# DefaultRui/VLN-VER

Hardware: AMD Instinct MI355X
Metric: viewpoints/sec (multi-view->voxel fwd+bwd), vocc.py config (higher is better)
Workload: dtype bf16

## Files before the change

### include/ver_ops.h

```cpp
#ifndef VER_OPS_H
#define VER_OPS_H

#include <stdint.h>

#ifdef __cplusplus
extern "C" {
#endif

#define VER_ABI_VERSION 31

#define VER_OK            0
#define VER_EINVAL       -1
#define VER_EUNSUPPORTED -2
#define VER_ELAUNCH      -3

#define VER_F32  0
#define VER_BF16 1

#define VER_I32  0
#define VER_I64  1

int         ver_abi_version(void);
const char* ver_last_error(void);

int ver_msda_forward(const float* value, const int64_t* shapes_hw, const int64_t* level_start,
                     const float* loc, const float* attn_w, float* out,
                     int B, int num_keys, int heads, int head_dim, int levels, int points,
                     int Nq, int im2col_step, void* stream);

int ver_msda_backward(const float* value, const int64_t* shapes_hw, const int64_t* level_start,
                      const float* loc, const float* attn_w, const float* grad_out,
                      float* grad_value, float* grad_loc, float* grad_attn_w,
                      int B, int num_keys, int heads, int head_dim, int levels, int points,
                      int Nq, int im2col_step, void* stream);

int ver_msda3d_forward(const float* value, const int64_t* shapes_dhw, const int64_t* level_start,
                       const float* loc, const float* attn_w, float* out,
                       int B, int num_keys, int heads, int head_dim, int levels, int points,
                       int Nq, void* stream);
int ver_msda3d_backward(const float* value, const int64_t* shapes_dhw, const int64_t* level_start,
                        const float* loc, const float* attn_w, const float* grad_out,
                        float* grad_value, float* grad_loc, float* grad_attn_w,
                        int B, int num_keys, int heads, int head_dim, int levels, int points,
                        int Nq, void* stream);


int ver_project_points(const float* world2pixel, const float* origin, const float* pc_range,
                       int B, int Ncam, int bev_z, int bev_h, int bev_w,
                       float img_w, float img_h,
                       float* uv, uint8_t* vis, int32_t* vis_list, int32_t* vis_cnt,
                       int32_t* zero_list, int32_t* zero_cnt, int32_t* fwd_list, int32_t* fwd_cnt,
                       void* stream);

int ver_hits_from_mask(const uint8_t* bev_mask, int B, int Ncam, int Nq, int D,
                       uint8_t* vis, int32_t* vis_list, int32_t* vis_cnt,
                       int32_t* zero_list, int32_t* zero_cnt, int32_t* fwd_list, int32_t* fwd_cnt,
                       void* stream);

#define VER_SCA_ROWS_PREZEROED 1
#define VER_SCA_VALUE_HEAD_MAJOR 2
#define VER_SCA_GRAD_SLOTS_BF16 4
int ver_sca_head_major_supported(int value_dtype, int head_dim, int points, int map_h, int map_w);
int ver_sca_zero_rows(const int32_t* zero_list, const int32_t* zero_cnt, float* slots, int B, int Nq, int row_floats,
                      void* stream);
int ver_sca_forward(const void* value, int value_dtype, const float* offsets, const float* logits,
                    const float* uv, const uint8_t* vis, const int32_t* vis_list,
                    const int32_t* vis_cnt, const int32_t* zero_list, const int32_t* zero_cnt,
                    const int32_t* fwd_list, const int32_t* fwd_cnt,
                    float* slots,
                    int B, int Ncam, int Nq, int D, int heads, int head_dim, int points,
                    int map_h, int map_w, int flags, void* stream);

int ver_sca_backward_grad_dtype(int value_dtype, int head_dim, int points, int map_h, int map_w);
int ver_sca_backward(const void* value, int value_dtype, const float* offsets, const float* logits,
                     const float* uv, const uint8_t* vis, const int32_t* vis_list,
                     const int32_t* vis_cnt, const int32_t* fwd_list, const int32_t* fwd_cnt,
                     const void* grad_slots,
                     void* grad_value, int grad_value_dtype, float* grad_offsets, float* grad_logits,
                     int B, int Ncam, int Nq, int D, int heads, int head_dim, int points,
                     int map_h, int map_w, int flags, void* stream);

int ver_lattice_im2col(const void* src, void* col, const int* taps, int ntaps,
                       int B, int Z, int H, int W, int C, int dtype, void* stream);
int ver_lattice_col2im(const void* grad_col, void* grad_src, const int* taps, int ntaps,
                       int B, int Z, int H, int W, int C, int dtype, void* stream);

int ver_lattice_gather(const void* src, void* col, const int* taps, const long* col_offset, long col_stride,
                       int ntaps, int B, int Zr, int Zs, int H, int W, int C, int layout, int dtype,
                       const void* const_rows, const long* const_offset, int const_blocks, int const_width, void* stream);
int ver_lattice_scatter(const void* grad_col, void* grad_src, const int* taps, const long* col_offset,
                        long col_stride, int ntaps, int B, int Zr, int Zs, int H, int W, int C, int layout, int dtype,
                        void* stream);

int ver_convt_weight_forward(const float* weight, void* taps, long pairs, int dtype, void* stream);
int ver_convt_weight_backward(const void* grad_taps, float* grad_weight, long pairs, int dtype, void* stream);
int ver_convt_weight_backward_blocks(const void* blocks, const long* block_offsets, long ld, const void* prev_bias,
                                     const void* grad_v, float* grad_weight, int ci, int co, int dtype, void* stream);
int ver_convt_weight_forward_blocks(const float* weight, const long* block_offsets, long ld, void* blocks, int ci, int co,
                                    int dtype, void* stream);
int ver_blocks_vec_forward(const void* blocks, const long* block_rows, int nblocks, long ld, int ci, int ncols, const float* x,
                           float* vec, int dtype, void* stream);
int ver_blocks_vec_backward(const void* blocks, const long* block_rows, int nblocks, long ld, int ci, int ncols,
                            const float* grad_vec, float* grad_x, int dtype, void* stream);
int ver_lattice_transpose(void* channels_last, void* channel_first, long cf_stride, int B, int Z, int H, int W,
                          int C, int layout, int to_channel_first, int dtype, void* stream);
int ver_lattice_rows(void* channels_last, void* rows, long quarter, int period, int nseg, const int* seg_off,
                     const int* seg_len, const long* seg_base, const int* seg_pitch, const int* seg_rows, int B, int Z,
                     int H, int W, int C, int layout, int to_rows, int dtype, void* stream);

int ver_ln_relu_forward(const void* x, const float* gamma, const float* beta, void* y,
                        float* mean, float* rstd, long N, int W, float eps, int dtype, void* stream);
int ver_ln_relu_backward(const void* x, const void* grad_y, const float* gamma, const float* beta,
                         const float* mean, const float* rstd, void* grad_x,
                         float* grad_gamma, float* grad_beta, long N, int W, int dtype, void* stream);

int ver_focal_loss_blocks(long N, int C);
int ver_focal_loss_forward(const void* logits, const int64_t* target, float* partial, long N, int C,
                           float gamma, float alpha, int dtype, int32_t* bad_labels, void* stream);
int ver_focal_loss_forward_grad(const void* logits, const int64_t* target, float* partial, void* grad, long N, int C,
                                float gamma, float alpha, int dtype, int32_t* bad_labels, void* stream);
int ver_focal_loss_forward_grad_u8(const void* logits, const uint8_t* target, float* partial, void* grad, long N, int C,
                                   float gamma, float alpha, int dtype, int32_t* bad_labels, void* stream);
int ver_focal_loss_backward(const void* logits, const int64_t* target, const float* scale, void* grad,
                            long N, int C, float gamma, float alpha, int dtype, void* stream);
int ver_focal_loss_forward_cw(const void* logits, const int64_t* target, const float* class_weight, float* partial,
                              long N, int C, float gamma, float alpha, int dtype, int32_t* bad_labels, void* stream);
int ver_focal_loss_forward_grad_cw(const void* logits, const int64_t* target, const float* class_weight, float* partial,
                                   void* grad, long N, int C, float gamma, float alpha, int dtype, int32_t* bad_labels,
                                   void* stream);
int ver_focal_loss_forward_grad_u8_cw(const void* logits, const uint8_t* target, const float* class_weight, float* partial,
                                      void* grad, long N, int C, float gamma, float alpha, int dtype, int32_t* bad_labels,
                                      void* stream);
int ver_focal_loss_backward_cw(const void* logits, const int64_t* target, const float* class_weight, const float* scale,
                               void* grad, long N, int C, float gamma, float alpha, int dtype, void* stream);
int ver_focal_loss_forward_u8(const void* logits, const uint8_t* target, float* partial, long N, int C,
                              float gamma, float alpha, int dtype, int32_t* bad_labels, void* stream);
int ver_focal_loss_backward_u8(const void* logits, const uint8_t* target, const float* scale, void* grad,
                               long N, int C, float gamma, float alpha, int dtype, void* stream);
int ver_focal_loss_forward_u8_cw(const void* logits, const uint8_t* target, const float* class_weight, float* partial,
                                 long N, int C, float gamma, float alpha, int dtype, int32_t* bad_labels, void* stream);
int ver_focal_loss_backward_u8_cw(const void* logits, const uint8_t* target, const float* class_weight, const float* scale,
                                  void* grad, long N, int C, float gamma, float alpha, int dtype, void* stream);

int ver_add_ln_forward(const void* a, int a_dtype, const float* residual, const float* gamma, const float* beta,
                       const int64_t* seed, float p_drop, float eps, float* y, void* y_bf16, float* mean,
                       float* rstd, long N, int C, void* stream);
int ver_add_ln_backward(const float* grad_y, const void* grad_y_bf16, const void* a, int a_dtype,
                        const float* residual, const float* gamma, const float* mean, const float* rstd,
                        const int64_t* seed, float p_drop, void* grad_a, float* grad_residual, float* grad_gamma,
                        float* grad_beta, long N, int C, void* stream);
int ver_relu_dropout_forward(const void* x, void* y, const int64_t* seed, float p_drop, long n, int dtype, void* stream);
int ver_relu_dropout_backward(const void* y, const void* grad_y, void* grad_x, float p_drop, long n, int dtype,
                              void* stream);

int ver_run_gather(const void* image, long image_stride, const int32_t* run_start, const int32_t* aug_idx,
                   void* rows, int B, int n_rows, int runs, int run_len, int n_aug, int row_elems, int dtype,
                   void* stream);
int ver_run_scatter(const void* rows, void* image, long image_stride, const int32_t* run_start, int B,
                    int n_rows, int runs, int run_len, int row_elems, int dtype, void* stream);

#define VER_OCC_MLP_CENTERED 2
long ver_occ_mlp_image_bytes(void);
int ver_occ_mlp_vector_floats(void);
int ver_occ_mlp_pack(const float* W1, const float* W2, const float* W3, void* image, void* stream);
int ver_occ_mlp_forward(const void* x, const void* image, const float* vectors, void* logits,
                        long N, int width, int classes, float eps, int flags, void* stream);
int ver_occ_mlp_forward_stats(const void* x, const void* image, const float* vectors, void* logits, float* rstd,
                              long N, int width, int classes, float eps, int flags, void* stream);
int ver_occ_mlp_backward(const void* x, const void* grad_logits, const void* image, const float* vectors,
                         void* grad_x, void* grad_a1, void* grad_a2, void* h1,
                         float* param_grads, long N, int width, int classes, float eps, int first_linear,
                         void* stream);
int ver_occ_mlp_backward_fused(const void* x, const void* grad_logits, const float* W2, const float* W3,
                               const float* vectors, void* grad_x, float* param_grads, long N, int width,
                               int classes, float eps, const float* grad_scale, int flags, void* stream);
int ver_occ_mlp_backward_fused_stats(const void* x, const void* grad_logits, const float* W2, const float* W3,
                                     const float* vectors, const float* rstd, void* grad_x, float* param_grads, long N,
                                     int width, int classes, float eps, const float* grad_scale, int flags, void* stream);
long ver_occ_mlp_backward_fused_slab_bytes(long N);
int ver_occ_mlp_backward_fused_slabs(const void* x, const void* grad_logits, const float* W2, const float* W3,
                                     const float* vectors, const float* rstd, void* grad_x, float* param_grads, float* slabs,
                                     long slab_bytes, long N, int width, int classes, float eps, const float* grad_scale,
                                     int flags, void* stream);

long ver_occ_predict_blocks(long N);
int  ver_occ_predict(const void* logits, int dtype, long N, int C, float threshold, int32_t* block_work,
                     int64_t* pairs, int64_t* count, void* stream);

int  ver_occ_confusion(const void* logits, int dtype, long rows_per_sample, int samples, int C, const uint8_t* labels,
                       const float* thresholds, int num_thresholds, int64_t* hist, void* stream);

int ver_occ_mlp_confusion(const void* x, const void* image, const float* vectors, const uint8_t* labels,
                          long rows_per_sample, int samples, const float* thresholds, int num_thresholds,
                          int64_t* hist, int width, int classes, float eps, int flags, void* stream);
int ver_occ_mlp_classes(const void* x, const void* image, const float* vectors, uint8_t* cls, float* prob,
                        long N, float threshold, int width, int classes, float eps, int flags, void* stream);

int  ver_wgrad_tn_splits(long M, int Ka, int N);
int  ver_wgrad_tn_splits_ld(long M, int Ka, int N, long ld);
long ver_wgrad_tn_workspace(long M, int Ka, int N, int splits);
int  ver_wgrad_tn(const void* a, long lda, const void* g, long ldg, long M, int Ka, int N, void* out, long ldo,
                  int out_dtype, int splits, int flags, void* workspace, long workspace_bytes, void* stream);
int  ver_wgrad_tn_segments(const void* lattice, int layout, int B, int H, int W, int C, const int* taps, int nseg, const void* cst,
                           int ncst, int cw, const void* g, long ldg, int N, void* out, long ldo, int out_dtype, int splits,
                           void* workspace, long workspace_bytes, void* stream);
int  ver_wgrad_tn_segments_splits(int B, int H, int W, long Ka, int N, long ldg);

int  ver_gemm_nn(const void* a, long lda, const void* w, long ldw, const float* bias, void* c, long ldc, long M, int K,
                 int N, int flags, void* stream);
int  ver_gemm_nn_taps(const void* lattice, int layout, int B, int H, int W, int C, const int* taps, int ntaps, const void* w,
                      long ldw, const float* rowpos, const float* bias, void* c, long ldc, int N, void* stream);
int  ver_gemm_nn_segments(const void* lattice, int layout, int B, int H, int W, int C, const int* taps, int ntaps,
                          const void* cst, int ncst, int cw, const void* w, long ldw, const float* rowpos, const float* bias,
                          void* c, long ldc, int N, void* stream);
int  ver_gemm_nn_planes(const void* lattice, int layout, int B, int H, int W, int C, long plane_elems, int nplanes,
                        const int* tap_plane, const int* taps, int ntaps, const void* cst, int ncst, int cw, const void* w,
                        long ldw, const float* rowpos, const float* bias, void* c, long ldc, int N, void* stream);
int  ver_gemm_nn_splits(long M, int K, int N);
int  ver_gemm_nn_splitk(const void* a, long lda, const void* w, long ldw, const float* bias, void* c, long ldc, long M, int K,
                        int N, int splits, void* workspace, long workspace_bytes, void* stream);

int ver_clip_adamw_step(void* const* table, const long* sizes, const int* chunk_tensor, const int* chunk_index,
                        int n_tensors, int n_chunks, int chunk_elems, float* partial, float* norm_out, float max_norm,
                        float lr, float beta1, float beta2, float eps, float weight_decay, long step, void* stream);

int ver_clip_adamw_step_tensors(void* const* table, const long* sizes, const int* chunk_tensor, const int* chunk_index,
                                const float* hyper, int* steps, int n_tensors, int n_chunks, int chunk_elems, float* partial,
                                float* norm_out, float max_norm, void* stream);

int ver_grad_pack(const void* const* table, const long* sizes, const long* offsets, const int* chunk_tensor,
                  const int* chunk_index, int n_tensors, int n_chunks, int chunk_elems, float scale, void* flat,
                  int flat_dtype, void* stream);

int ver_clip_adamw_step_flat(void* const* table, const long* sizes, const long* offsets, const int* chunk_tensor,
                             const int* chunk_index, const float* hyper, int* steps, const void* flat, int flat_dtype,
                             int n_tensors, int n_chunks, int chunk_elems, float* partial, float* norm_out, float max_norm,
                             void* stream);

int ver_lsa_solve(const float* cost, const int32_t* ncols, int32_t* match, int32_t* bad,
                  int P, int R, int Ccap, void* stream);

int ver_box3d_overlaps(const float* a, const int32_t* na, const float* b, const int32_t* nb, float* iou,
                       int S, int Acap, int Bcap, void* stream);

int ver_det_match(const float* pred_boxes, const int32_t* pred_labels, const float* pred_scores,
                  const uint8_t* pred_valid, const float* gt_boxes, const int32_t* gt_labels, const int32_t* ngt,
                  const float* thresholds, int num_thresholds, float* iou_max, int32_t* gt_index,
                  uint8_t* tp_bits, int64_t* npos, int num_classes, int S, int Pcap, int Gcap, void* stream);

int ver_det_costs(const void* cls, int cls_dtype, const float* box, int box_ld, const float* gt,
                  const int64_t* gt_labels, const int32_t* counts, float* cost, int L, int B, int Q, int C, int Gcap,
                  float w_cls, float alpha, float gamma, float eps, float w_reg, void* stream);
int ver_det_set_loss_forward(const void* cls, int cls_dtype, const float* box, int box_ld, const int32_t* match,
                             const float* gt, const int64_t* gt_labels, const int32_t* counts,
                             const float* code_weights, float* sums, int32_t* npos, int32_t* bad, int L, int B, int Q,
                             int C, int Gcap, float alpha, float gamma, void* stream);
int ver_det_set_loss_backward(const void* cls, int cls_dtype, const float* box, int box_ld, const int32_t* match,
                              const float* gt, const int64_t* gt_labels, const int32_t* counts,
                              const float* code_weights, const float* scale, void* grad_cls, float* grad_box, int L,
                              int B, int Q, int C, int Gcap, float alpha, float gamma, void* stream);

int ver_det_decode(const void* cls, int cls_dtype, const float* box, int box_ld, float* out_boxes, float* out_scores,
                   int32_t* out_labels, uint8_t* out_valid, int32_t* out_query, const float* center_range,
                   float score_threshold, int flags, int B, int Q, int C, int K, int codes, void* stream);

int ver_occ_targets(const void* pairs, int pair_dtype, const int32_t* offsets, long n_total, const void* invalid,
                    int invalid_dtype, const int32_t* invalid_offsets, long n_invalid, const int32_t* row_table,
                    uint8_t* labels, int32_t* count, int32_t* bad, long voxel_num, int zdim, int classes, int bs,
                    void* stream);

int ver_dattn3d_supported(int B, int num_keys, int heads, int head_dim, int levels, int points, int Nq);
int ver_dattn3d_forward(const void* value, int value_dtype, const int64_t* shapes_dhw, const int64_t* level_start,
                        const float* ref, const void* offsets, const void* logits, int q_dtype, void* out, int out_dtype,
                        int B, int num_keys, int heads, int head_dim, int levels, int points, int Nq, void* stream);
int ver_dattn3d_backward(const void* value, int value_dtype, const int64_t* shapes_dhw, const int64_t* level_start,
                         const float* ref, const void* offsets, const void* logits, int q_dtype, const void* grad_out,
                         int out_dtype, void* grad_value, void* grad_offsets, void* grad_logits, float* grad_ref,
                         int B, int num_keys, int heads, int head_dim, int levels, int points, int Nq, void* stream);

int ver_mha_supported(int B, int heads, int head_dim, int Nq, int Nk);
int ver_mha_forward(const void* q, const void* k, const void* v, int dtype, long ldq, long ldk, long ldv,
                    const int64_t* seed, float p_drop, void* out, float* lse, int B, int heads, int head_dim, int Nq, int Nk,
                    void* stream);
int ver_mha_backward(const void* q, const void* k, const void* v, int dtype, long ldq, long ldk, long ldv,
                     const void* grad_out, const float* lse, const int64_t* seed, float p_drop, void* grad_q, void* grad_k,
                     void* grad_v, long ldgq, long ldgk, long ldgv, int B, int heads, int head_dim, int Nq, int Nk,
                     void* stream);

#ifdef __cplusplus
}
#endif
#endif
```

### vln-ver_amd/csrc/ver_wgrad.hip

```cpp
#include "ver_gemm_tile.h"

namespace {
using namespace gemm_tile;

constexpr int kSlabRows = 16;
constexpr int kSlabBytes = 2 * kSlabRows * kTile * 2;
constexpr int kRing = 8;
constexpr int kLdsBytes = kRing * kSlabBytes;
constexpr int kPhaseSlabs = 2;
constexpr int kAhead = 4;
static_assert(kAhead >= kPhaseSlabs && kAhead + 4 <= kRing, "prefetch distance against the ring (WAR on the slot)");

struct WgradArgs {
    const __bf16* A;
    const __bf16* G;
    float* ws;
    long lda, ldg, M, Mc;
    int S, Ka, N, tiles_n, T;
    void* out;
    long ldo;
    int out_bf16;
    const __bf16* lattice;
    long lattice_bytes;
    const __bf16* cst;
    long cst_bytes;
    int B, H, W, C, P, CW, ncst, nseg;
    int seg_start[65];
    signed char kind[64], dz[64], dy[64], dx[64];
};

struct WTapLane {
    int taddr;
    int boff;
    int bstep;
    int pend;
    int tend;
    int rows_left;
    int vo;
    int taddr1, pend1, vo1;
};

template <int L>
__device__ __forceinline__ int wtap_table_entry(const WgradArgs& t, int seg, int pos) {
    if (seg < 0) return kOutside;
    if (t.kind[seg]) return (pos * t.ncst + t.dz[seg]) * t.CW * 2;
    const int hw = t.H * t.W;
    const int zl = pos / hw, rem = pos - zl * hw;
    const int y = rem / t.W, x = rem - y * t.W;
    return cell_off<L>(LatticeGeom{t.B, t.H, t.W, t.C}, 0, zl, y + t.dy[seg], x + t.dx[seg], t.dz[seg]);
}

__device__ __forceinline__ int lds_read_b32(int addr) {
    int v;
    asm volatile("ds_read_b32 %0, %1" : "=v"(v) : "v"(addr) : "memory");
    return v;
}

__device__ __forceinline__ void wtap_step(const WgradArgs& t, WTapLane& tl, int tfetched) {
    tl.boff += tl.pend;
    tl.rows_left -= kSlabRows;
    tl.vo = tl.rows_left > 0 ? (int)((unsigned)tfetched + (unsigned)tl.boff) : kOutside;
    tl.taddr += 4 * kSlabRows;
    tl.pend = 0;
    if (tl.taddr >= tl.tend) tl.taddr -= 4 * t.P, tl.pend = tl.bstep;
}

__device__ __forceinline__ void wtap_step2(const WgradArgs& t, WTapLane& tl, int tfetched0, int tfetched1) {
    tl.boff += tl.pend;
    tl.rows_left -= kSlabRows;
    tl.vo = tl.rows_left > 0 ? (int)((unsigned)tfetched0 + (unsigned)tl.boff) : kOutside;
    tl.boff += tl.pend1;
    tl.rows_left -= kSlabRows;
    tl.vo1 = tl.rows_left > 0 ? (int)((unsigned)tfetched1 + (unsigned)tl.boff) : kOutside;
    tl.taddr = tl.taddr1 + 4 * kSlabRows;
    tl.pend = 0;
    if (tl.taddr >= tl.tend) tl.taddr -= 4 * t.P, tl.pend = tl.bstep;
    tl.taddr1 = tl.taddr + 4 * kSlabRows;
    tl.pend1 = 0;
    if (tl.taddr1 >= tl.tend) tl.taddr1 -= 4 * t.P, tl.pend1 = tl.bstep;
}

struct WgradLane {
    int offA[4], offB[4];
    int voA, voG;
    int stepA, stepG;
    int dmaoff;
};

template <int PS, int IMPL>
__device__ __forceinline__ void phase(char* lds, f32x4 (&acc)[8][4], const WgradLane& c, __amdgpu_buffer_rsrc_t ra,
                                      __amdgpu_buffer_rsrc_t rg, unsigned& soA, unsigned& soG, const WgradArgs& t, WTapLane& tl) {
    constexpr int SB = ((2 * PS) & 3) * kSlabBytes;
    constexpr int UP = 2 * PS >= 4 ? 65536 : 0;
    i32x2 al[8], ah[8], bl[4], bh[4];
    int tn0 = 0, tn1 = 0;
#pragma unroll
    for (int q = 0; q < 4; ++q) {
        const int a = c.offA[q] + UP, b = c.offB[q] + UP;
        al[q] = tr_read<SB>(a);
        ah[q] = tr_read<SB + 512>(a);
        bl[q] = tr_read<SB>(b);
        bh[q] = tr_read<SB + 512>(b);
        al[4 + q] = tr_read<SB + 1024>(a);
        ah[4 + q] = tr_read<SB + 1536>(a);
    }
#pragma unroll
    for (int u = 0; u < 2; ++u) {
        const int ds = (2 * PS + u + kAhead) % kRing;
        if constexpr (IMPL < 0) {
            __builtin_amdgcn_raw_ptr_buffer_load_lds(ra, (lds_void*)(lds + ds * kSlabBytes + c.dmaoff), 16, c.voA, (int)soA, 0, 0);
        } else {
            __builtin_amdgcn_raw_ptr_buffer_load_lds(ra, (lds_void*)(lds + ds * kSlabBytes + c.dmaoff), 16, u ? tl.vo1 : tl.vo, 0, 0, 0);
            if (u) tn1 = lds_read_b32(tl.taddr1);
            else tn0 = lds_read_b32(tl.taddr);
        }
        __builtin_amdgcn_raw_ptr_buffer_load_lds(rg, (lds_void*)(lds + ds * kSlabBytes + kSlabBytes / 2 + c.dmaoff), 16, c.voG, (int)soG, 0, 0);
        soA += (unsigned)c.stepA;
        soG += (unsigned)c.stepG;
    }
    asm volatile("s_waitcnt vmcnt(%0)" ::"n"(2 * (kAhead - kPhaseSlabs)) : "memory");
    __builtin_amdgcn_s_barrier();
    asm volatile("s_waitcnt lgkmcnt(0)"
                 : "+v"(al[0]), "+v"(ah[0]), "+v"(al[1]), "+v"(ah[1]), "+v"(al[2]), "+v"(ah[2]), "+v"(al[3]), "+v"(ah[3]), "+v"(al[4]),
                   "+v"(ah[4]), "+v"(al[5]), "+v"(ah[5]), "+v"(al[6]), "+v"(ah[6]), "+v"(al[7]), "+v"(ah[7]), "+v"(bl[0]), "+v"(bh[0]),
                   "+v"(bl[1]), "+v"(bh[1]), "+v"(bl[2]), "+v"(bh[2]), "+v"(bl[3]), "+v"(bh[3]), "+v"(tn0), "+v"(tn1)
                 :
                 : "memory");
    bf16x8 a[8], b[4];
#pragma unroll
    for (int i = 0; i < 8; ++i) a[i] = frag(al[i], ah[i]);
#pragma unroll
    for (int j = 0; j < 4; ++j) b[j] = frag(bl[j], bh[j]);
    __builtin_amdgcn_sched_barrier(0);
    __builtin_amdgcn_s_setprio(1);
#pragma unroll
    for (int it = 0; it < 8; ++it)
#pragma unroll
        for (int jt = 0; jt < 4; ++jt)
            acc[it][jt] = __builtin_amdgcn_mfma_f32_16x16x32_bf16(a[it], b[jt], acc[it][jt], 0, 0, 0);
    __builtin_amdgcn_s_setprio(0);
    __builtin_amdgcn_sched_barrier(0);
    if constexpr (IMPL >= 0) {
        wtap_step2(t, tl, tn0, tn1);
        __builtin_amdgcn_sched_barrier(0);
    }
    __builtin_amdgcn_s_barrier();
}

template <int PS, int IMPL>
__device__ __forceinline__ void phases_from(int left, char* lds, f32x4 (&acc)[8][4], const WgradLane& c,
                                            __amdgpu_buffer_rsrc_t ra, __amdgpu_buffer_rsrc_t rg, unsigned& soA, unsigned& soG,
                                            const WgradArgs& t, WTapLane& tl) {
    if constexpr (PS < kRing / kPhaseSlabs) {
        if (left > PS * kPhaseSlabs) {
            phase<PS, IMPL>(lds, acc, c, ra, rg, soA, soG, t, tl);
            phases_from<PS + 1, IMPL>(left, lds, acc, c, ra, rg, soA, soG, t, tl);
        }
    }
}

template <int IMPL>
__device__ __forceinline__ void wgrad_body(const WgradArgs& p) {
    extern __shared__ __attribute__((aligned(1024))) char lds[];
    const int tid = threadIdx.x, lane = tid & 63;
    const int wave = __builtin_amdgcn_readfirstlane(tid >> 6);
    const int wr = wave >> 2, wc = wave & 3;
    int chunk, tile;
    {
        const int b = blockIdx.x;
        if ((p.S & 7) == 0) {
            const int xcd = b & 7, idx = b >> 3;
            chunk = xcd + 8 * (idx / p.T);
            tile = idx % p.T;
        } else {
            chunk = b / p.T;
            tile = b % p.T;
        }
    }
    const int mt = tile / p.tiles_n, nt = tile - mt * p.tiles_n;
    const long row0 = (long)chunk * p.Mc;
    const long rows = max(0L, min(p.Mc, p.M - row0));
    const int nslab = (int)((rows + kSlabRows * kPhaseSlabs - 1) / (kSlabRows * kPhaseSlabs)) * kPhaseSlabs;

    const __bf16* ab = IMPL < 0 ? p.A + row0 * p.lda + (long)mt * kTile : nullptr;
    const __bf16* gb = p.G + row0 * p.ldg + (long)nt * kTile;
    const long abytes = ((p.M - row0 - 1) * p.lda + p.Ka - (long)mt * kTile) * 2;
    const long gbytes = ((p.M - row0 - 1) * p.ldg + p.N - (long)nt * kTile) * 2;
    const __amdgpu_buffer_rsrc_t rg = __builtin_amdgcn_make_buffer_rsrc((void*)gb, 0, (int)max(0L, min(gbytes, 0xFFFFFFFFL)), 0x00020000);
    WgradLane c;
    const int prow = lane >> 3, pch = (lane & 7) ^ Shape::swz(prow, wave >> 2);
    WTapLane tl = {};
    bool a_cst = false;
    if constexpr (IMPL >= 0) {
        int* tables = reinterpret_cast<int*>(lds + kLdsBytes);
        auto seg_of = [&](int col0) {
            int seg = -1;
            for (int i = 0; i < p.nseg; ++i)
                if (col0 >= p.seg_start[i] && col0 < p.seg_start[i + 1]) seg = i;
            return seg;
        };
        for (int q = 0; q < 4; ++q) {
            const int seg = seg_of(mt * kTile + 64 * q);
            for (int i = tid; i < p.P; i += 512) tables[q * p.P + i] = wtap_table_entry<IMPL>(p, seg, i);
        }
        __syncthreads();
        const int col0 = mt * kTile + 64 * (wave & 3);
        const int seg = seg_of(col0);
        a_cst = seg >= 0 && p.kind[seg];
        const long r = row0 + 8 * (wave >> 2) + prow;
        const int b0 = (int)(r / p.P), pos0 = (int)(r - (long)b0 * p.P);
        tl.bstep = a_cst ? 0 : (IMPL == 3 ? p.H * p.W : 4 * p.H * p.W) * p.C * 2;
        tl.boff = b0 * tl.bstep + (seg < 0 ? 0 : (col0 - p.seg_start[seg]) * 2) + pch * 16;
        const int lbase = (int)(uintptr_t)(__attribute__((address_space(3))) char*)(lds + kLdsBytes) + (wave & 3) * p.P * 4;
        tl.tend = lbase + 4 * p.P;
        tl.taddr = lbase + 4 * pos0;
        tl.pend = 0;
        tl.rows_left = (int)min(min(p.M, row0 + p.Mc) - r, 0x7FFFFFF0L) + kSlabRows;
        int t0 = lds_read_b32(tl.taddr);
        asm volatile("s_waitcnt lgkmcnt(0)" : "+v"(t0)::"memory");
        wtap_step(p, tl, t0);
    }
    const __amdgpu_buffer_rsrc_t ra =
        IMPL < 0 ? __builtin_amdgcn_make_buffer_rsrc((void*)ab, 0, (int)max(0L, min(abytes, 0xFFFFFFFFL)), 0x00020000)
                 : __builtin_amdgcn_make_buffer_rsrc((void*)(a_cst ? p.cst : p.lattice), 0,
                                                     (int)max(0L, min(a_cst ? p.cst_bytes : p.lattice_bytes, 0x7FFFFFFFL)), 0x00020000);
    c.voA = (int)(((8 * (wave >> 2) + prow) * p.lda + 64 * (wave & 3)) * 2) + pch * 16;
    c.voG = (int)(((8 * (wave >> 2) + prow) * p.ldg + 64 * (wave & 3)) * 2) + pch * 16;
    c.stepA = (int)(kSlabRows * p.lda * 2);
    c.stepG = (int)(kSlabRows * p.ldg * 2);
    c.dmaoff = wave * 1024;
    unsigned soA = 0, soG = 0;

    {
        const int g = lane >> 4, cl = lane & 15;
        const int lbase = (int)(uintptr_t)(__attribute__((address_space(3))) char*)lds;
#pragma unroll
        for (int q = 0; q < 4; ++q) {
            const int ch = (2 * q + ((cl & 3) >> 1)) ^ Shape::swz(cl >> 2, g & 1);
            const int rowoff = lbase + (g >> 1) * kSlabBytes + (g & 1) * 4096 + (cl >> 2) * 128 + ch * 16 + (cl & 1) * 8;
            c.offA[q] = rowoff + 2 * wr * 1024;
            c.offB[q] = rowoff + wc * 1024 + kSlabBytes / 2;
        }
    }

    Shape::acc_t acc[Shape::NI][Shape::NJ];
#pragma unroll
    for (int it = 0; it < Shape::NI; ++it)
#pragma unroll
        for (int jt = 0; jt < Shape::NJ; ++jt)
#pragma unroll
            for (int r = 0; r < Shape::NR; ++r) acc[it][jt][r] = 0.0f;

#pragma unroll
    for (int s = 0; s < kAhead; ++s) {
        if constexpr (IMPL < 0) {
            __builtin_amdgcn_raw_ptr_buffer_load_lds(ra, (lds_void*)(lds + s * kSlabBytes + c.dmaoff), 16, c.voA, (int)soA, 0, 0);
        } else {
            __builtin_amdgcn_raw_ptr_buffer_load_lds(ra, (lds_void*)(lds + s * kSlabBytes + c.dmaoff), 16, tl.vo, 0, 0, 0);
            int tn = lds_read_b32(tl.taddr);
            asm volatile("s_waitcnt lgkmcnt(0)" : "+v"(tn)::"memory");
            wtap_step(p, tl, tn);
        }
        __builtin_amdgcn_raw_ptr_buffer_load_lds(rg, (lds_void*)(lds + s * kSlabBytes + kSlabBytes / 2 + c.dmaoff), 16, c.voG, (int)soG, 0, 0);
        soA += (unsigned)c.stepA;
        soG += (unsigned)c.stepG;
    }
    if constexpr (IMPL >= 0) {
        const int vo0 = tl.vo;
        int tn = lds_read_b32(tl.taddr);
        asm volatile("s_waitcnt lgkmcnt(0)" : "+v"(tn)::"memory");
        wtap_step(p, tl, tn);
        tl.vo1 = tl.vo;
        tl.vo = vo0;
        tl.taddr1 = tl.taddr + 4 * kSlabRows;
        tl.pend1 = 0;
        if (tl.taddr1 >= tl.tend) tl.taddr1 -= 4 * p.P, tl.pend1 = tl.bstep;
    }
    asm volatile("s_waitcnt vmcnt(%0)" ::"n"(2 * (kAhead - kPhaseSlabs)) : "memory");
    __builtin_amdgcn_s_barrier();
    if (wr == 1) __builtin_amdgcn_s_barrier();

    int s = 0;
    for (; s + kRing <= nslab; s += kRing) phases_from<0, IMPL>(kRing, lds, acc, c, ra, rg, soA, soG, p, tl);
    phases_from<0, IMPL>(nslab - s, lds, acc, c, ra, rg, soA, soG, p, tl);
    if (wr == 0) __builtin_amdgcn_s_barrier();
    asm volatile("s_waitcnt vmcnt(0)" ::: "memory");

    const int i0 = mt * kTile + 128 * wr + Shape::lane_row(lane), j0 = nt * kTile + 64 * wc + (lane & (Shape::TW - 1));
    if (p.S == 1 && p.out) {
#pragma unroll
        for (int it = 0; it < Shape::NI; ++it)
#pragma unroll
            for (int jt = 0; jt < Shape::NJ; ++jt) {
                const int j = j0 + Shape::TW * jt;
#pragma unroll
                for (int r = 0; r < Shape::NR; ++r) {
                    const int i = i0 + Shape::TW * it + Shape::reg_row(r);
                    if (i < p.Ka && j < p.N) {
                        if (p.out_bf16)
                            reinterpret_cast<__bf16*>(p.out)[(long)i * p.ldo + j] = (__bf16)acc[it][jt][r];
                        else
                            reinterpret_cast<float*>(p.out)[(long)i * p.ldo + j] = acc[it][jt][r];
                    }
                }
            }
        return;
    }
    float* out = p.ws + (long)chunk * p.Ka * p.N;
#pragma unroll
    for (int it = 0; it < Shape::NI; ++it)
#pragma unroll
        for (int jt = 0; jt < Shape::NJ; ++jt) {
            const int j = j0 + Shape::TW * jt;
#pragma unroll
            for (int r = 0; r < Shape::NR; ++r) {
                const int i = i0 + Shape::TW * it + Shape::reg_row(r);
                if (i < p.Ka && j < p.N) out[(long)i * p.N + j] = acc[it][jt][r];
            }
        }
}

__global__ __launch_bounds__(512) void k_wgrad_tn(WgradArgs p) {
    wgrad_body<-1>(p);
}

template <int L>
__global__ __launch_bounds__(512) void k_wgrad_tn_seg(WgradArgs p) {
    wgrad_body<L>(p);
}

template <typename OT>
__global__ __launch_bounds__(256) void k_wgrad_reduce(const float* __restrict__ ws, OT* __restrict__ out, long ldo, int S,
                                                      int Ka, int N) {
    const long n4 = (long)Ka * N / 4;
    const long stride = (long)Ka * N;
    for (long e = blockIdx.x * 256L + threadIdx.x; e < n4; e += (long)gridDim.x * 256) {
        float4 acc = *reinterpret_cast<const float4*>(ws + 4 * e);
        for (int s = 1; s < S; ++s) {
            const float4 v = *reinterpret_cast<const float4*>(ws + s * stride + 4 * e);
            acc.x += v.x;
            acc.y += v.y;
            acc.z += v.z;
            acc.w += v.w;
        }
        const long i = (4 * e) / N, j = (4 * e) - i * N;
        OT* o = out + i * ldo + j;
        if constexpr (sizeof(OT) == 4) {
            *reinterpret_cast<float4*>(o) = acc;
        } else {
            typedef __bf16 bf16x4 __attribute__((ext_vector_type(4)));
            bf16x4 v;
            v.x = (__bf16)acc.x;
            v.y = (__bf16)acc.y;
            v.z = (__bf16)acc.z;
            v.w = (__bf16)acc.w;
            *reinterpret_cast<bf16x4*>(o) = v;
        }
    }
}

long max_chunk_rows(long ld) {
    if (ld <= 0) return 45000;
    const long rows = (0xFFFFFFFFL / (ld * 2)) - 16 * kRing - 2 * kSlabRows - 1;
    return rows < 45000 ? (rows > 2 * kSlabRows ? rows : 2 * kSlabRows) : 45000;
}

int pick_splits(long M, int Ka, int N, long ld = 0) {
    const long cap = max_chunk_rows(ld);
    const long tiles = (long)((Ka + kTile - 1) / kTile) * ((N + kTile - 1) / kTile);
    static const int cand[] = {1, 2, 3, 4, 6, 8, 12, 16, 24, 32, 48, 64};
    int best = 0;
    double best_us = 0.0;
    for (int s : cand) {
        if ((M + s - 1) / s > cap) continue;
        if (s > 1 && M / s < 256) break;
        if (M > 32768 && s % 8) continue;
        const long rounds = (tiles * s + 255) / 256;
        const double slabs = (double)((M + s - 1) / s + 15) / 16.0;
        double us = (double)rounds * (slabs * 0.37 + 8.0) + (s == 1 ? 0.25 : (double)s) * (double)Ka * (double)N * 8.0 / 3.0e6;
        if (s % 8 == 0) us *= 0.97;
        if (!best || us < best_us) {
            best = s;
            best_us = us;
        }
    }
    if (!best) {
        best = 64;
        while (best < 65536 && (M + best - 1) / best > cap) best *= 2;
    }
    return best;
}

int launch_wgrad(const char* who, WgradArgs& p, int layout, long M, long Ka, int N, void* out, long ldo, int out_dtype, int splits,
                 void* workspace, long workspace_bytes, hipStream_t st) {
    const long ld = p.lda > p.ldg ? p.lda : p.ldg;
    const int S = splits > 0 ? splits : pick_splits(M, (int)Ka, N, ld);
    VER_REQUIRE(S <= 65536, VER_EINVAL, "%s: %d row chunks", who, S);
    const long Mc = ((M + S - 1) / S + 2 * kSlabRows - 1) / (2 * kSlabRows) * (2 * kSlabRows);
    VER_REQUIRE((Mc + 16 * kRing) * ld * 2 < 0xFFFFFFFFL, VER_EUNSUPPORTED,
                "%s: a row chunk exceeds the 4-GiB range of a buffer offset (more splits)", who);
    VER_REQUIRE(workspace_bytes >= (long)S * Ka * N * (long)sizeof(float), VER_EINVAL, "%s: workspace of %ld bytes, %ld needed", who,
                workspace_bytes, (long)S * Ka * N * (long)sizeof(float));
    p.ws = (float*)workspace;
    p.M = M;
    p.Mc = Mc;
    p.S = S;
    p.Ka = (int)Ka;
    p.N = N;
    p.tiles_n = (N + kTile - 1) / kTile;
    p.T = (int)((Ka + kTile - 1) / kTile) * p.tiles_n;
    const bool direct = S == 1 && M > 0;
    p.out = direct ? out : nullptr;
    p.ldo = ldo;
    p.out_bf16 = out_dtype == VER_BF16;
    if (M > 0) {
        const auto kern = layout < 0 ? k_wgrad_tn : layout == 0 ? k_wgrad_tn_seg<0> : layout == 2 ? k_wgrad_tn_seg<2> : k_wgrad_tn_seg<3>;
        const int ldsb = layout < 0 ? kLdsBytes : kLdsBytes + 4 * p.P * 4;
        if (int rc = launch_tile_kernel(who, kern, p, p.T * S, ldsb, st)) return rc;
    } else if (int zrc = ver_zero_async(workspace, (size_t)S * Ka * N * sizeof(float), st)) {
        return zrc;
    }
    if (direct) return ver_check_launch(who);
    const long n4 = Ka * N / 4;
    long grid = (n4 + 255) / 256;
    if (grid > 8192) grid = 8192;
    if (out_dtype == VER_F32)
        hipLaunchKernelGGL(k_wgrad_reduce<float>, dim3((unsigned)grid), dim3(256), 0, st, (const float*)workspace, (float*)out, ldo, S, (int)Ka, N);
    else
        hipLaunchKernelGGL(k_wgrad_reduce<__bf16>, dim3((unsigned)grid), dim3(256), 0, st, (const float*)workspace, (__bf16*)out, ldo, S, (int)Ka, N);
    return ver_check_launch(who);
}
}

extern "C" int ver_wgrad_tn_splits(long M, int Ka, int N) {
    if (M <= 0 || Ka <= 0 || N <= 0) return 1;
    return pick_splits(M, Ka, N);
}

extern "C" int ver_wgrad_tn_splits_ld(long M, int Ka, int N, long ld) {
    if (M <= 0 || Ka <= 0 || N <= 0) return 1;
    return pick_splits(M, Ka, N, ld);
}

extern "C" long ver_wgrad_tn_workspace(long M, int Ka, int N, int splits) {
    if (Ka <= 0 || N <= 0) return 0;
    if (splits <= 0) splits = ver_wgrad_tn_splits(M, Ka, N);
    return (long)splits * Ka * N * (long)sizeof(float);
}

extern "C" int ver_wgrad_tn(const void* a, long lda, const void* g, long ldg, long M, int Ka, int N, void* out, long ldo,
                            int out_dtype, int splits, int flags, void* workspace, long workspace_bytes, void* stream) {
    VER_REQUIRE(M >= 0 && Ka > 0 && N > 0, VER_EINVAL, "ver_wgrad_tn: bad sizes M=%ld Ka=%d N=%d", M, Ka, N);
    VER_REQUIRE(out && workspace && ((a && g) || M == 0), VER_EINVAL, "ver_wgrad_tn: null pointer argument");
    VER_REQUIRE(out_dtype == VER_F32 || out_dtype == VER_BF16, VER_EINVAL, "ver_wgrad_tn: out_dtype %d", out_dtype);
    VER_REQUIRE(flags == 0, VER_EINVAL, "ver_wgrad_tn: unknown flags 0x%x", flags);
    VER_REQUIRE(lda >= Ka && ldg >= N && ldo >= N, VER_EINVAL, "ver_wgrad_tn: row pitch smaller than the row");
    VER_REQUIRE(lda % 8 == 0 && ldg % 8 == 0 && ((uintptr_t)a & 15) == 0 && ((uintptr_t)g & 15) == 0, VER_EUNSUPPORTED,
                "ver_wgrad_tn: operands must be 16-byte aligned with row pitches that are multiples of 8 elements");
    VER_REQUIRE(N % 4 == 0 && ldo % 4 == 0 && ((uintptr_t)out & 15) == 0, VER_EUNSUPPORTED,
                "ver_wgrad_tn: N and the output pitch must be multiples of 4");
    WgradArgs p = {};
    p.A = (const __bf16*)a;
    p.G = (const __bf16*)g;
    p.lda = lda;
    p.ldg = ldg;
    return launch_wgrad("ver_wgrad_tn", p, -1, M, Ka, N, out, ldo, out_dtype, splits, workspace, workspace_bytes, (hipStream_t)stream);
}

extern "C" int ver_wgrad_tn_segments(const void* lattice, int layout, int B, int H, int W, int C, const int* taps, int nseg,
                                     const void* cst, int ncst, int cw, const void* g, long ldg, int N, void* out, long ldo,
                                     int out_dtype, int splits, void* workspace, long workspace_bytes, void* stream) {
    if (int rc = check_lattice_args("ver_wgrad_tn_segments", layout, B, H, W, C, N, nseg)) return rc;
    VER_REQUIRE(out && workspace && ((lattice && g && taps) || B == 0), VER_EINVAL, "ver_wgrad_tn_segments: null pointer argument");
    VER_REQUIRE(out_dtype == VER_F32 || out_dtype == VER_BF16, VER_EINVAL, "ver_wgrad_tn_segments: out_dtype %d", out_dtype);
    VER_REQUIRE(nseg <= 64, VER_EUNSUPPORTED, "ver_wgrad_tn_segments: %d segments (at most 64)", nseg);
    VER_REQUIRE(C % 64 == 0 && (cst == nullptr || (ncst > 0 && ncst <= 64 && cw > 0 && cw % 64 == 0 && ((uintptr_t)cst & 15) == 0)),
                VER_EUNSUPPORTED, "ver_wgrad_tn_segments: segment widths (C = %d, pattern blocks of %d) must be multiples of 64", C, cw);
    const long M = (long)B * 2 * H * W, lbytes = (long)B * 4 * H * W * C * 2;
    const int P = 2 * H * W;
    VER_REQUIRE(P >= kSlabRows && P <= 2048 && lbytes < 0x7FFFFFFFL, VER_EUNSUPPORTED,
                "ver_wgrad_tn_segments: %d rows per viewpoint / a source lattice of %ld bytes (16 <= rows <= 2048: four offset tables "
                "next to the 128-KB ring in LDS; below 2 GiB)", P, lbytes);
    VER_REQUIRE(ldg >= N && ldo >= N && ldg % 8 == 0 && ((uintptr_t)g & 15) == 0 && ((uintptr_t)lattice & 15) == 0, VER_EUNSUPPORTED,
                "ver_wgrad_tn_segments: g must be 16-byte aligned with a row pitch that is a multiple of 8 elements");
    VER_REQUIRE(N % 4 == 0 && ldo % 4 == 0 && ((uintptr_t)out & 15) == 0, VER_EUNSUPPORTED,
                "ver_wgrad_tn_segments: N and the output pitch must be multiples of 4");
    long Ka = 0;
    if (int rc = check_segments("ver_wgrad_tn_segments", "ver_wgrad_tn_segments", taps, nseg, C, cst, ncst, cw, &Ka)) return rc;
    VER_REQUIRE(Ka < 0x7FFFFFFFL, VER_EUNSUPPORTED, "ver_wgrad_tn_segments: %ld columns", Ka);
    WgradArgs p = {};
    for (int i = 0, col = 0; i < nseg; ++i) {
        const int dz = taps[3 * i];
        p.seg_start[i] = col;
        p.kind[i] = dz < 0;
        p.dz[i] = (signed char)(dz < 0 ? -1 - dz : dz);
        if (dz >= 0) p.dy[i] = (signed char)taps[3 * i + 1], p.dx[i] = (signed char)taps[3 * i + 2];
        col += dz < 0 ? cw : C;
    }
    p.seg_start[nseg] = (int)Ka;
    p.G = (const __bf16*)g;
    p.ldg = ldg;
    p.lattice = (const __bf16*)lattice;
    p.lattice_bytes = lbytes;
    p.cst = (const __bf16*)cst;
    p.cst_bytes = cst ? (long)P * ncst * cw * 2 : 0;
    p.B = B, p.H = H, p.W = W, p.C = C, p.P = P, p.CW = cw, p.ncst = ncst, p.nseg = nseg;
    return launch_wgrad("ver_wgrad_tn_segments", p, layout, M, Ka, N, out, ldo, out_dtype, splits, workspace, workspace_bytes,
                        (hipStream_t)stream);
}

extern "C" int ver_wgrad_tn_segments_splits(int B, int H, int W, long Ka, int N, long ldg) {
    const long M = (long)B * 2 * H * W;
    if (M <= 0 || Ka <= 0 || N <= 0) return 1;
    return pick_splits(M, (int)Ka, N, ldg);
}
```

### vln-ver_amd/dense_heads/row_linear.py

```python
import torch
import torch.nn.functional as F

_CHUNK = 8000


class _RowLinear(torch.autograd.Function):

    @staticmethod
    def forward(ctx, x, weight, bias):
        w = weight.to(x.dtype)
        ctx.save_for_backward(x, w)
        ctx.has_bias = bias is not None
        ctx.weight_dtype = weight.dtype
        if bias is None:
            return x @ w.t()
        return torch.addmm(bias.to(x.dtype), x, w.t())

    @staticmethod
    def backward(ctx, g):
        x, w = ctx.saved_tensors
        g = g.contiguous()
        n, o = g.shape
        gx = g @ w if ctx.needs_input_grad[0] else None
        gb = None
        if ctx.has_bias:
            gb = g.sum(0, dtype=torch.float32)
        if g.dtype == torch.bfloat16 and x.dtype == torch.bfloat16 and n >= 4096 and min(o, x.shape[1]) >= 192:
            from ..hipops import wgrad_tn, wgrad_tn_supported
            if wgrad_tn_supported(g, x):
                wide = torch.float32 if ctx.weight_dtype == torch.float32 else torch.bfloat16
                if wide == torch.bfloat16 and gb is not None:
                    gb = gb.to(torch.bfloat16)
                return gx, wgrad_tn(g, x, out_dtype=wide), gb
        s = n // _CHUNK
        main = s * _CHUNK
        gw = x.new_zeros((o, x.shape[1]), dtype=torch.float32)
        if s:
            g3 = g[:main].view(s, _CHUNK, o)
            gw += torch.bmm(g3.transpose(1, 2), x[:main].view(s, _CHUNK, -1)).sum(0, dtype=torch.float32)
        if main < n:
            gw += (g[main:].t() @ x[main:]).float()
        return gx, gw, gb


def row_linear(x, weight, bias):
    if not x.is_cuda:
        return F.linear(x, weight, bias)
    if torch.is_autocast_enabled('cuda'):
        x = x.to(torch.get_autocast_dtype('cuda'))
    shape = x.shape
    with torch.autocast('cuda', enabled=False):
        y = _RowLinear.apply(x.reshape(-1, shape[-1]), weight, bias)
    return y.view(*shape[:-1], -1)
```

### vln-ver_amd/dense_heads/upsample.py

```python
import os

import torch

from . import _cpu_algebra
from ._cpu_algebra import ZS_PLAIN, ZS_PLANAR_SPLIT, ZS_SPLIT, planar_to_plain, planar_zs_to_plain, zs_to_plain
from ._cpu_algebra import plain_to_planar
from .lattice_plan import (_CLASSES, _COLS3, _COLS4, _PW, _PW2, _aug_rows_z4, _block_offsets, _class_patterns, _class_rows_z4,
                           _class_segments_z4, _const_rows_z4, _dgrad_plan, _layer0_z4_plan, _layer_plan, _layer_plan_z4,
                           _stack_tables_z4)

KERNEL = (3, 5, 5)
GEOM = dict(stride=(1, 2, 2), padding=(2, 4, 4), dilation=(2, 2, 2), output_padding=(0, 1, 1))
_HIP_DTYPES = (torch.float32, torch.bfloat16)


class _HipAlgebra:

    @staticmethod
    def corr_weight(weight, dtype):
        if weight.dtype == torch.float32 and dtype in _HIP_DTYPES:
            from ..hipops import convt_weight_taps
            return convt_weight_taps(weight, dtype)
        return _cpu_algebra.corr_weight(weight, dtype)

# ... 85 lines not shown
    d_k = torch.addcmul(d_rows[:n_data].view(75, ci, co), prev_bias.to(dt)[None, :, None], d_v[:, None, :])
    d_prev = torch.bmm(k, d_v.unsqueeze(2)).sum(0).squeeze(1)
    return d_k, d_vaug[75].to(prev_bias.dtype), d_prev.to(prev_bias.dtype)


def _layer0(e, k, bias):
    b, z, h, w, c = e.shape
    taps = [(2 * a - 2, bb - 2, cc - 2) for a in range(3) for bb in range(5) for cc in range(5)]
    a_mat = _im2col(e, taps)
    out = torch.addmm(bias, a_mat, k.reshape(75 * c, -1))
    return out.view(b, z, h, w, -1)


def _gather27(e, planar, a_mat, ci, hc, wc):
    _algebra(e).gather27(e, planar, a_mat, ci, hc, wc, _COLS3.taps, _COLS3.block_offsets(ci))


def _scatter27(d_a, planar, shape, ci, hc, wc):
    return _algebra(d_a).scatter27(d_a, planar, shape, ci, hc, wc, _COLS3.taps, _COLS3.block_offsets(ci))


class _LatticeLayer(torch.autograd.Function):

    @staticmethod
    def forward(ctx, e, k, bias, prev_bias, planar):
        if planar:
            _, b, z, hh, wh, ci = e.shape
            hc, wc = 2 * hh, 2 * wh
        else:
            b, z, hc, wc, ci = e.shape
        co = k.shape[-1]
        plan, kt, total_rows = _layer_plan(ci, e.device)
        m = b * z * hc * wc
        a_mat = e.new_empty(m, kt)
        _gather27(e, planar, a_mat, ci, hc, wc)
        a3 = a_mat.view(b, z * hc * wc, kt)
        for cls, pat in zip(_CLASSES, _class_patterns(z, hc, wc, e.device, e.dtype)):
            o = _COLS3.const_offset(cls, ci)
            a3[:, :, o:o + _PW] = pat
        rows = _stacked_rows(k, bias, prev_bias, total_rows)
        out = e.new_empty(4, m, co)
        for p, cls in enumerate(_CLASSES):
            c0, c1, ridx = plan[cls]
            torch.mm(a_mat[:, c0:c1], rows.index_select(0, ridx), out=out[p])
        ctx.save_for_backward(a_mat, rows, k, prev_bias)
        ctx.geom = (planar, tuple(e.shape), hc, wc)
        return out.view(4, b, z, hc, wc, co)

    @staticmethod
    def backward(ctx, grad_out):
        a_mat, rows, k, prev_bias = ctx.saved_tensors
        planar, e_shape, hc, wc = ctx.geom
        _, ci, co = k.shape
        plan, kt, total_rows = _layer_plan(ci, a_mat.device)
        m = a_mat.shape[0]
        g = grad_out.contiguous().view(4, m, co)
        d_a = a_mat.new_empty(m, kt)
        d_a[:, kt - _PW:] = 0
        d_rows = rows.new_empty(total_rows, co)
        for p, cls in enumerate(_CLASSES):
            c0, c1, ridx = plan[cls]
            w = rows.index_select(0, ridx)
            if p == 0:
                torch.mm(g[p], w.t(), out=d_a[:, c0:c1])
            else:
                torch.addmm(d_a[:, c0:c1], g[p], w.t(), out=d_a[:, c0:c1])
            d_rows.index_copy_(0, ridx, rows_tn(a_mat[:, c0:c1], g[p]))
        d_e = _scatter27(d_a, planar, e_shape, ci, hc, wc)
        return (d_e, *_stacked_rows_backward(d_rows, k, prev_bias), None)


def _gather_z4(e, layout, a_mat, taps, offs, ci, hc, wc, with_const=False):
    const = _const_rows_z4(ci, hc, wc, e.device, e.dtype) if with_const else None
    return _algebra(e).gather_z4(e, layout, a_mat, taps, offs, ci, hc, wc, const)


def _scatter_z4(d_a, layout, shape, taps, offs, ci, hc, wc):
    return _algebra(d_a).scatter_z4(d_a, layout, shape, taps, offs, ci, hc, wc)


_IMPLICIT_TAPS = os.environ.get('VER_IMPLICIT_TAPS', '1') != '0'


def _implicit_taps(e, layout, rows, combined_hw, ci, raw, const_width):
    if not (_IMPLICIT_TAPS and _OWN_GEMM and raw is not None and _on_hip(e) and e.dtype == torch.bfloat16 and rows >= _OWN_GEMM_MIN_ROWS):
        return False
    from ..hipops import gemm_nn_taps_supported, wgrad_tn_segments_supported
    return gemm_nn_taps_supported(e, layout, None, ci) and wgrad_tn_segments_supported(e, layout, combined_hw, ci, const_width, None)


def _dgrad_implicit(kind, g_planes, weights, b, hc, wc, ci, co):
    from ..hipops import gemm_nn_taps
    lat = g_planes.view(g_planes.shape[0], b, 2, hc, wc, 2, co)
    rows, taps, planes, nb = _dgrad_plan(kind, ci, g_planes.device)
    wcat = weights.index_select(0, rows).view(nb, 2 * ci, 2 * co).transpose(1, 2).reshape(nb * 2 * co, 2 * ci)
    d_e = gemm_nn_taps(lat if kind != 'l0' else lat[0], ZS_SPLIT, (hc, wc), taps, wcat, planes=planes if kind != 'l0' else None,
                       timer_class='head_gemm_dgrad')
    return d_e.view(b, 2, hc, wc, 2, ci)


def _dgrad_explicit_l0(g, wmat, shape, taps, offs, ci, h, w):
    with gemm_timed('head_gemm_dgrad', g.shape[0], g.shape[1], wmat.shape[0]):
        d_a = torch.mm(g, wmat.t())
    return _scatter_z4(d_a, ZS_PLAIN, shape, taps, offs, ci, h, w)


class _Layer0Z4Taps(torch.autograd.Function):

    @staticmethod
    def forward(ctx, x, k, bias):
        b, _, h, w, ci = x.shape
        co = k.shape[-1]
        taps, offs, lo, hi = _layer0_z4_plan(ci, x.device)
        a_mat = x.new_empty(b * 2 * h * w, 50 * ci)
        _gather_z4(x, ZS_PLAIN, a_mat, taps, offs, ci, h, w)
        rows = k.reshape(75 * ci, co)
        wmat = torch.cat([rows.index_select(0, lo), rows.index_select(0, hi)], 1)
        out = mm_fwd(a_mat, wmat, bias=torch.cat([bias, bias]))
        ctx.save_for_backward(a_mat, wmat)
        ctx.geom = (tuple(x.shape), ci, co, h, w)
        return out.view(b, 2, h, w, 2, co)

    @staticmethod
    def backward(ctx, grad_out):
        a_mat, wmat = ctx.saved_tensors
        shape, ci, co, h, w = ctx.geom
        taps, offs, lo, hi = _layer0_z4_plan(ci, a_mat.device)
        g = grad_out.contiguous().view(-1, 2 * co)
        d_x = _dgrad_explicit_l0(g, wmat, shape, taps, offs, ci, h, w)
        d_w = rows_tn(a_mat, g)
        d_b = g.sum(0, dtype=torch.float64 if g.dtype == torch.float64 else torch.float32)
        d_lo = d_w.new_zeros(75 * ci, co)
        d_hi = d_w.new_zeros(75 * ci, co)
        d_lo.index_copy_(0, lo, d_w[:, :co])
        d_hi.index_copy_(0, hi, d_w[:, co:])
        return d_x, (d_lo + d_hi).view(75, ci, co), (d_b[:co] + d_b[co:]).to(g.dtype)


class _Layer0Z4Raw(torch.autograd.Function):

    @staticmethod
    def forward(ctx, x, raw, bias):
        from ..hipops import convt_weight_forward_blocks
        b, _, h, w, ci = x.shape
        co = raw.shape[1]
        taps, offs, _, _ = _layer0_z4_plan(ci, x.device)
        ctx.implicit = _implicit_taps(x, ZS_PLAIN, b * 2 * h * w, (h, w), ci, raw, 0)
        if ctx.implicit:
            operand = x.contiguous()
        else:
            operand = x.new_empty(b * 2 * h * w, 50 * ci)
            _gather_z4(x, ZS_PLAIN, operand, taps, offs, ci, h, w)
        wmat = convt_weight_forward_blocks(raw, _block_offsets('l0', ci, co, x.device), x.new_empty(50 * ci, 2 * co), ci, co)
        bias2 = torch.cat([bias, bias])
        if ctx.implicit:
            from ..hipops import gemm_nn_taps
            out = gemm_nn_taps(operand, ZS_PLAIN, (h, w), taps, wmat, bias=bias2.to(x.dtype).float())
        else:
            out = mm_fwd(operand, wmat, bias=bias2)
        ctx.save_for_backward(operand, wmat)
        ctx.geom = (tuple(x.shape), ci, co, h, w)
        return out.view(b, 2, h, w, 2, co)

    @staticmethod
    def backward(ctx, grad_out):
        from ..hipops import convt_weight_backward_blocks
        operand, wmat = ctx.saved_tensors
        shape, ci, co, h, w = ctx.geom
        taps, offs, _, _ = _layer0_z4_plan(ci, operand.device)
        g = grad_out.contiguous().view(-1, 2 * co)
        if ctx.implicit:
            from ..hipops import wgrad_tn_segments
            d_x = zs_to_plain(_dgrad_implicit('l0', g[None], wmat, shape[0], h, w, ci, co))
            d_w = wgrad_tn_segments(operand, ZS_PLAIN, (h, w), taps, g)
        else:
            d_x = _dgrad_explicit_l0(g, wmat, shape, taps, offs, ci, h, w)
            d_w = rows_tn(operand, g)
        d_b = g.sum(0, dtype=torch.float32)
        d_raw = convt_weight_backward_blocks(d_w, _block_offsets('l0', ci, co, d_w.device), None, None, ci, co)
        return d_x, d_raw, (d_b[:co] + d_b[co:]).to(g.dtype)


def _geom_z4(e, planar):
    if planar:
        _, b, _, hh, wh, _, ci = e.shape
        return ZS_PLANAR_SPLIT, b, 2 * hh, 2 * wh, ci
    b, _, hc, wc, _, ci = e.shape
    return ZS_SPLIT, b, hc, wc, ci


def _tap_matrix_z4(e, layout, b, hc, wc, ci):
    _, kt, _, taps, offs = _layer_plan_z4(ci, e.device)
    a_mat = e.new_empty(b * 2 * hc * wc, kt)
    if not _gather_z4(e, layout, a_mat, taps, offs, ci, hc, wc, with_const=True):
        a3 = a_mat.view(b, 2 * hc * wc, kt)
        for cls, pat in zip(_CLASSES, _class_patterns(4, hc, wc, e.device, e.dtype)):
            o = _COLS4.const_offset(cls, ci)
            halves = pat.view(2, 2 * hc * wc, _PW)
            a3[:, :, o:o + _PW] = halves[0]
            a3[:, :, o + _PW:o + _PW2] = halves[1]
    return a_mat


def _class_ranges_z4(ci, device):
    plan, rows = _layer_plan_z4(ci, device)[0], _class_rows_z4(ci)
    ranges = [(plan[cls][0], plan[cls][1], rows[cls][0], rows[cls][0] + plan[cls][1] - plan[cls][0]) for cls in _CLASSES]
    return ranges, ranges[-1][3]


def _dgrad_class(d_a, p, g_p, w, c0, c1):
    with gemm_timed('head_gemm_dgrad', g_p.shape[0], g_p.shape[1], c1 - c0):
        if p == 0:
            torch.mm(g_p, w.t(), out=d_a[:, c0:c1])
        else:
            torch.addmm(d_a[:, c0:c1], g_p, w.t(), out=d_a[:, c0:c1])


class _LatticeLayerZ4Taps(torch.autograd.Function):

    @staticmethod
    def forward(ctx, e, k, bias, prev_bias, planar):
        layout, b, hc, wc, ci = _geom_z4(e, planar)
        co = k.shape[-1]
        plan, _, total_rows, _, _ = _layer_plan_z4(ci, e.device)
        a_mat = _tap_matrix_z4(e, layout, b, hc, wc, ci)
        out = e.new_empty(4, a_mat.shape[0], 2 * co)
        rows = _stacked_rows(k, bias, prev_bias, total_rows)
        ws = []
        for p, cls in enumerate(_CLASSES):
            c0, c1, _, _, lohi = plan[cls]
            ws.append(rows.index_select(0, lohi).view(c1 - c0, 2 * co))
            mm_fwd(a_mat[:, c0:c1], ws[p], out=out[p])
        ctx.save_for_backward(a_mat, k, prev_bias, *ws)
        ctx.geom = (layout, tuple(e.shape), hc, wc)
        return out.view(4, b, 2, hc, wc, 2, co)

    @staticmethod
    def backward(ctx, grad_out):
        a_mat, k, prev_bias, *ws = ctx.saved_tensors
        layout, e_shape, hc, wc = ctx.geom
        _, ci, co = k.shape
        plan, kt, total_rows, taps, offs = _layer_plan_z4(ci, a_mat.device)
        m = a_mat.shape[0]
        g = grad_out.contiguous().view(4, m, 2 * co)
        d_a = a_mat.new_empty(m, kt)
        d_a[:, kt - _PW2:] = 0
        d_lo = a_mat.new_zeros(total_rows, co)
        d_hi = a_mat.new_zeros(total_rows, co)
        for p, cls in enumerate(_CLASSES):
            c0, c1, lo, hi, _ = plan[cls]
            _dgrad_class(d_a, p, g[p], ws[p], c0, c1)
            d_w = rows_tn(a_mat[:, c0:c1], g[p])
            d_lo.index_copy_(0, lo, d_w[:, :co])
            d_hi.index_copy_(0, hi, d_w[:, co:])
        d_e = _scatter_z4(d_a, layout, e_shape, taps, offs, ci, hc, wc)
        del d_a
        return (d_e, *_stacked_rows_backward(d_lo + d_hi, k, prev_bias), None)


class _LatticeLayerZ4Raw(torch.autograd.Function):

    @staticmethod
    def forward(ctx, e, raw, bias, prev_bias, planar):
        from ..hipops import blocks_vec_forward, convt_weight_forward_blocks
        layout, b, hc, wc, ci = _geom_z4(e, planar)
        co = raw.shape[1]
        dt = e.dtype
        m = b * 2 * hc * wc
        ctx.implicit = _implicit_taps(e, layout, m, (hc, wc), ci, raw, _PW2)
        operand = e.contiguous() if ctx.implicit else _tap_matrix_z4(e, layout, b, hc, wc, ci)
        out = e.new_empty(4, m, 2 * co)
        ranges, n_rows = _class_ranges_z4(ci, e.device)
        block_rows, tap_slot, const_rows, const_src = _stack_tables_z4(ci, e.device)
        stack = e.new_empty(n_rows, 2 * co)
        convt_weight_forward_blocks(raw, _block_offsets('lat', ci, co, e.device), stack, ci, co)
        v = blocks_vec_forward(stack, block_rows, ci, prev_bias).view(-1, co).index_select(0, tap_slot)
        vaug = torch.cat([v.to(dt), bias.to(dt)[None], v.new_zeros(_PW - 75, co, dtype=dt)])
        stack.view(-1, co).index_copy_(0, const_rows, vaug.index_select(0, const_src))
        for p, (cls, (c0, c1, r0, r1)) in enumerate(zip(_CLASSES, ranges)):
            if ctx.implicit:
                from ..hipops import gemm_nn_taps
                gemm_nn_taps(operand, layout, (hc, wc), _class_segments_z4(cls, ci), stack[r0:r1],
                             const_rows=_const_rows_z4(ci, hc, wc, e.device, dt)[0], out=out[p])
            else:
                mm_fwd(operand[:, c0:c1], stack[r0:r1], out=out[p])
        ctx.save_for_backward(operand, stack, prev_bias)
        ctx.geom = (layout, tuple(e.shape), b, hc, wc, ci, co)
        return out.view(4, b, 2, hc, wc, 2, co)

    @staticmethod
    def backward(ctx, grad_out):
        from ..hipops import blocks_vec_backward, convt_weight_backward_blocks
        operand, stack, prev_bias = ctx.saved_tensors
        layout, e_shape, b, hc, wc, ci, co = ctx.geom
        _, kt, _, taps, offs = _layer_plan_z4(ci, operand.device)
        ranges, n_rows = _class_ranges_z4(ci, operand.device)
        dt = operand.dtype
        m = b * 2 * hc * wc
        g = grad_out.contiguous().view(4, m, 2 * co)
        if not ctx.implicit:
            d_a = operand.new_empty(m, kt)
            d_a[:, kt - _PW2:] = 0
        d_stack = operand.new_empty(n_rows, 2 * co)
        for p, (cls, (c0, c1, r0, r1)) in enumerate(zip(_CLASSES, ranges)):
            if ctx.implicit:
                from ..hipops import wgrad_tn_segments
                wgrad_tn_segments(operand, layout, (hc, wc), _class_segments_z4(cls, ci), g[p], out=d_stack[r0:r1],
                                  const_rows=_const_rows_z4(ci, hc, wc, operand.device, dt)[0])
            else:
                _dgrad_class(d_a, p, g[p], stack[r0:r1], c0, c1)
                rows_tn(operand[:, c0:c1], g[p], out=d_stack[r0:r1])
        if ctx.implicit:
            d_e = _dgrad_implicit('lat', g, stack, b, hc, wc, ci, co)
            if layout == ZS_PLANAR_SPLIT:
                d_e = d_e.view(b, 2, hc // 2, 2, wc // 2, 2, 2, ci).permute(3, 5, 0, 1, 2, 4, 6, 7).reshape(e_shape)
        else:
            d_e = _scatter_z4(d_a, layout, e_shape, taps, offs, ci, hc, wc)
            del d_a
        own = d_stack.view(-1, co).index_select(0, _aug_rows_z4(ci, d_stack.device)).view(8, _PW, co)
        d_vaug = own.sum(0, dtype=torch.float32)
        d_v = d_vaug[:75].to(dt)
        pb = prev_bias.to(dt)
        d_raw = convt_weight_backward_blocks(d_stack, _block_offsets('lat', ci, co, d_stack.device), pb, d_v, ci, co)
        block_rows, tap_slot, _, _ = _stack_tables_z4(ci, d_stack.device)
        dv2 = d_vaug.new_zeros(2 * block_rows.numel(), co).index_copy_(0, tap_slot, d_vaug[:75])
        d_prev = blocks_vec_backward(stack, block_rows, ci, dv2.view(block_rows.numel(), 2 * co))
        return d_e, d_raw, d_vaug[75].to(prev_bias.dtype), d_prev.to(prev_bias.dtype), None


class _Layer0Z4:

    @staticmethod
    def apply(x, k, bias, raw=None):
        return _Layer0Z4Taps.apply(x, k, bias) if raw is None else _Layer0Z4Raw.apply(x, raw, bias)


class _LatticeLayerZ4:

    @staticmethod
    def apply(e, k, bias, prev_bias, planar, raw=None):
        if raw is None:
            return _LatticeLayerZ4Taps.apply(e, k, bias, prev_bias, planar)
        return _LatticeLayerZ4Raw.apply(e, raw, bias, prev_bias, planar)


def gemm_timed(name, m, k, n):
    from ..hipops import timed
    return timed(name, 2.0 * m * k * n)


_OWN_GEMM = os.environ.get('VER_OWN_GEMM', '1') == '1'
_OWN_GEMM_MIN_ROWS = int(os.environ.get('VER_OWN_GEMM_MIN_ROWS', '14000'))
_OWN_GEMM_SKINNY_ROWS = 2048


def mm_fwd(a, w, out=None, bias=None):
    m, k = a.shape
    n = w.shape[1]
    if _OWN_GEMM and _on_hip(a) and a.dtype == torch.bfloat16 and w.dtype == torch.bfloat16 and k >= 2048 and \
            (m >= _OWN_GEMM_MIN_ROWS or m <= _OWN_GEMM_SKINNY_ROWS):
        from ..hipops import gemm_nn, gemm_nn_splits, gemm_nn_supported
        if gemm_nn_supported(a, w) and (out is None or (out.stride(-1) == 1 and out.dtype == torch.bfloat16)) and \
                (m >= _OWN_GEMM_MIN_ROWS or gemm_nn_splits(m, k, n) > 1):
            return gemm_nn(a, w, None if bias is None else bias.to(a.dtype).float(), out)
    with gemm_timed('head_gemm_fwd', m, k, n):
        if bias is None:
            return torch.mm(a, w, out=out) if out is not None else torch.mm(a, w)
        b = bias.to(a.dtype)
        return torch.addmm(b, a, w, out=out) if out is not None else torch.addmm(b, a, w)


def rows_tn(a, g, out_dtype=None, out=None):
    if _on_hip(a) and a.dtype == torch.bfloat16 and g.dtype == torch.bfloat16:
        from ..hipops import wgrad_tn, wgrad_tn_supported
        if g.stride(-1) != 1 or g.stride(0) % 8:
            g = g.contiguous()
        if wgrad_tn_supported(a, g):
            return wgrad_tn(a, g, out_dtype=out_dtype if out is None else out.dtype, out=out)
    if out is not None:
        return torch.mm(a.t(), g, out=out) if out.dtype == a.dtype else out.copy_(torch.mm(a.t(), g))
    res = torch.mm(a.t(), g)
    return res if out_dtype is None else res.to(out_dtype)


def _compute_dtype(x):
    if _on_hip(x) and torch.is_autocast_enabled('cuda'):
        return torch.get_autocast_dtype('cuda')
    return x.dtype


class _ChannelsLast(torch.autograd.Function):

    @staticmethod
    def forward(ctx, x0, dt, split):
        from ..hipops import lattice_transpose
        b, c, z, h, w = x0.shape
        cf = x0.to(dt).contiguous().view(b, c * z * h * w)
        e = torch.empty(b, z, h, w, c, dtype=dt, device=x0.device)
        lattice_transpose(e.view(b, 1, split[0], split[1], c), cf, split, 0, False)
        ctx.split, ctx.in_dtype = split, x0.dtype
        return e

    @staticmethod
    def backward(ctx, g):
        from ..hipops import lattice_transpose
        b, z, h, w, c = g.shape
        g = g.contiguous()
        cf = torch.empty(b, c * z * h * w, dtype=g.dtype, device=g.device)
        lattice_transpose(g.view(b, 1, ctx.split[0], ctx.split[1], c), cf, ctx.split, 0, True)
        return cf.view(b, c, z, h, w).to(ctx.in_dtype), None, None


def _channels_last(x0, dt):
    return _algebra(x0).channels_last(x0, dt)


def upsample_lattice(x0, weights, biases):
    dt = _compute_dtype(x0)
    e = _channels_last(x0, dt)
    bs = [b.to(dt) for b in biases]
    if e.shape[1] == 4 and _on_hip(e) and dt in _HIP_DTYPES and all(_on_hip(w) and w.dtype == torch.float32 for w in weights):
        e = _Layer0Z4.apply(e, None, bs[0], weights[0])
        e = _LatticeLayerZ4.apply(e, None, bs[1], bs[0], False, weights[1])
        e = _LatticeLayerZ4.apply(e, None, bs[2], bs[1], True, weights[2])
        return e, bs[2]
    ks = [_corr_weight(w, dt) for w in weights]
    if e.shape[1] == 4:
        e = _Layer0Z4.apply(e, ks[0], bs[0])
        e = _LatticeLayerZ4.apply(e, ks[1], bs[1], bs[0], False)
        e = _LatticeLayerZ4.apply(e, ks[2], bs[2], bs[1], True)
        return e, bs[2]
    e = _layer0(e, ks[0], bs[0])
    e = _LatticeLayer.apply(e, ks[1], bs[1], bs[0], False)
    e = _LatticeLayer.apply(e, ks[2], bs[2], bs[1], True)
    return e, bs[2]


def full_volume(e, bias):
    if e.dim() == 7:
        e = planar_zs_to_plain(e)
    elif e.dim() == 6:
        e = planar_to_plain(e)
    b, z, h, w, c = e.shape
    y = bias.view(1, c, 1, 1, 1).expand(b, c, z, 2 * h, 2 * w).contiguous()
    y[:, :, :, ::2, ::2] = e.permute(0, 4, 1, 2, 3)
    return y


def upsample_dense(x0, weights, biases):
    e, b = upsample_lattice(x0, weights, biases)
    return full_volume(e, b)
```

### vln-ver_amd/hipops.py

```python
import ctypes
import os
import re

import torch
from torch.autograd import Function
from torch.autograd.function import once_differentiable

_PKG = os.path.dirname(os.path.abspath(__file__))
LIB_PATH = os.environ.get('VER_HIP_LIB') or os.path.join(_PKG, 'libver_hip.so')
ABI_VERSION = 31
HEADER = os.path.join(os.path.dirname(_PKG), 'include', 'ver_ops.h')
_PARAMS = {'int': ctypes.c_int, 'long': ctypes.c_long, 'float': ctypes.c_float}
_RETURNS = {'int': ctypes.c_int, 'long': ctypes.c_long, 'const char*': ctypes.c_char_p}


class HipLibraryError(RuntimeError):
    pass


def prototypes(path=HEADER):
    if not os.path.exists(path):
        raise HipLibraryError('%s not found: the C ABI is bound from its prototypes' % path)
    text = re.sub(r'/\*.*?\*/|//[^\n]*|^\s*#[^\n]*', ' ', open(path).read(), flags=re.S | re.M)
    out = {}
# ... 1515 lines not shown
    what = 'det_match'
    pred_boxes, gt_boxes = _boxes7(pred_boxes, 'pred_boxes', what), _boxes7(gt_boxes, 'gt_boxes', what)
    s, p = pred_boxes.shape[:2]
    g = gt_boxes.shape[1]
    dev = pred_boxes.device
    pred_labels = _gpu(pred_labels, 'pred_labels', torch.int32)
    pred_scores = _gpu(pred_scores, 'pred_scores', torch.float32)
    pred_valid = _gpu(pred_valid, 'pred_valid', torch.uint8)
    gt_labels = _gpu(gt_labels, 'gt_labels', torch.int32)
    for name, t, shape in (('pred_labels', pred_labels, (s, p)), ('pred_scores', pred_scores, (s, p)),
                           ('pred_valid', pred_valid, (s, p)), ('gt_boxes', gt_boxes, (s, g, 7)), ('gt_labels', gt_labels, (s, g))):
        if tuple(t.shape) != shape or t.device != dev:
            raise ValueError('%s: %s must be %s on %s, got %s on %s' % (what, name, shape, dev, tuple(t.shape), t.device))
    ngt = _counts(ngt, 'ngt', what, s, dev)
    if ngt is None:
        raise ValueError('det_match: ngt is required')
    thr = [float(t) for t in thresholds]
    if not 1 <= len(thr) <= DET_MATCH_MAX_THRESHOLDS:
        raise ValueError('det_match: %d thresholds (1..%d)' % (len(thr), DET_MATCH_MAX_THRESHOLDS))
    if npos.dim() != 1 or npos.dtype != torch.int64 or not npos.is_contiguous() or npos.device != dev or npos.numel() < 1:
        raise ValueError('det_match: npos must be a contiguous int64 [num_classes] tensor on %s' % (dev,))
    if p < 1 or p > DET_MATCH_MAX_BOXES or g > DET_MATCH_MAX_BOXES or p * g > DET_MATCH_MAX_PAIRS:
        raise ValueError('det_match: P=%d G=%d (1 <= P <= %d, G <= %d, P * G <= %d)'
                         % (p, g, DET_MATCH_MAX_BOXES, DET_MATCH_MAX_BOXES, DET_MATCH_MAX_PAIRS))
    iou_max = torch.empty(s, p, dtype=torch.float32, device=dev)
    gt_index = torch.empty(s, p, dtype=torch.int32, device=dev)
    tp_bits = torch.empty(s, p, dtype=torch.uint8, device=dev)
    if s:
        host_thr = (ctypes.c_float * len(thr))(*thr)
        _launch('ver_det_match', lambda: lib().ver_det_match(
            _p(pred_boxes), _p(pred_labels), _p(pred_scores), _p(pred_valid), _p(gt_boxes), _p(gt_labels), _p(ngt), host_thr,
            len(thr), _p(iou_max), _p(gt_index), _p(tp_bits), _p(npos), npos.numel(), s, p, g, _stream()))
    return iou_max, gt_index, tp_bits


DET_DECODE_MAX_SLOTS = 1024
DET_DECODE_MAX_KEYS = 16384


def det_decode(cls, box, center_range, score_threshold=None, bottom_center=True, k=None):
    what = 'det_decode'
    if not box.is_cuda:
        raise RuntimeError('box must be a GPU tensor: the VER ops only exist as HIP kernels')
    if box.dtype != torch.float32:
        raise TypeError('box must be %s, got %s' % (torch.float32, box.dtype))
    if box.dim() != 3 or box.shape[-1] not in (8, 10) or box.shape[1] < 1:
        raise ValueError('%s: box must be [B, Q >= 1, 8 | 10] normalised codes, got %s' % (what, tuple(box.shape)))
    bs, nq, codes = box.shape
    if not (box.stride(2) == 1 and box.stride(1) >= codes and (bs <= 1 or box.stride(0) == nq * box.stride(1))):
        box = box.contiguous()
    ld, dev = box.stride(1), box.device
    ncls, code = 0, 0
    if cls is not None:
        cls = _gpu(cls, 'cls')
        if cls.dtype not in (torch.float32, torch.bfloat16):
            raise TypeError('%s: cls must be float32 or bfloat16, got %s' % (what, cls.dtype))
        if cls.dim() != 3 or tuple(cls.shape[:2]) != (bs, nq) or cls.shape[2] < 1 or cls.device != dev:
            raise ValueError('%s: cls must be [%d, %d, C >= 1] on %s, got %s on %s' % (what, bs, nq, dev, tuple(cls.shape), cls.device))
        ncls, code = cls.shape[2], 1 if cls.dtype == torch.bfloat16 else 0
        keys = nq * ncls
        k = min(keys, DET_DECODE_MAX_SLOTS) if k is None else int(k)
    else:
        keys = nq
        k = nq if k is None else int(k)
        if k != nq:
            raise ValueError('%s: the layout form decodes every query: k=%d, Q=%d' % (what, k, nq))
    if not 1 <= k <= min(keys, DET_DECODE_MAX_SLOTS) or keys > DET_DECODE_MAX_KEYS:
        raise ValueError('%s: k=%d Q*C=%d (1 <= k <= min(Q*C, %d), Q*C <= %d)' % (what, k, keys, DET_DECODE_MAX_SLOTS, DET_DECODE_MAX_KEYS))
    rng = [float(v) for v in center_range]
    if len(rng) != 6:
        raise ValueError('%s: center_range holds %d numbers (6)' % (what, len(rng)))
    flags = (1 if bottom_center else 0) | (2 if score_threshold is not None else 0)
    boxes = torch.empty(bs, k, codes - 1, dtype=torch.float32, device=dev)
    scores = torch.empty(bs, k, dtype=torch.float32, device=dev)
    labels = torch.empty(bs, k, dtype=torch.int32, device=dev)
    valid = torch.empty(bs, k, dtype=torch.uint8, device=dev)
    query = torch.empty(bs, k, dtype=torch.int32, device=dev)
    if bs:
        host_rng = (ctypes.c_float * 6)(*rng)
        _launch('ver_det_decode', lambda: lib().ver_det_decode(
            _p(cls), code, _p(box), ld, _p(boxes), _p(scores), _p(labels), _p(valid), _p(query), host_rng,
            float(score_threshold or 0.0), flags, bs, nq, ncls, k, codes, _stream()))
    return boxes, scores, labels, valid, query


def _occ_offsets(offsets, n, name):
    import numpy as np
    off = np.asarray(offsets)
    if off.ndim != 1 or off.size < 1 or not np.issubdtype(off.dtype, np.integer):
        raise ValueError('%s must be an integer [bs + 1] array' % name)
    if off[0] != 0 or off[-1] != n or (np.diff(off) < 0).any():
        raise ValueError('%s must ascend from 0 to %d' % (name, n))
    return off.astype(np.int64)


def occ_targets_host(pairs, offsets, voxel_num, zdim, classes, row_table=None, invalid=None, invalid_offsets=None):
    import numpy as np
    voxel_num, zdim, classes = int(voxel_num), int(zdim), int(classes)
    if not 1 <= classes < 255 or zdim < 1 or voxel_num < 0 or voxel_num % zdim:
        raise ValueError('occ_targets_host: voxel_num=%d zdim=%d classes=%d (1 <= classes < 255, voxel_num %% zdim == 0)'
                         % (voxel_num, zdim, classes))
    pairs = np.asarray(pairs).reshape(-1, 2).astype(np.int64)
    off = _occ_offsets(offsets, pairs.shape[0], 'offsets')
    bs = off.size - 1
    if bs * voxel_num >= 2 ** 31:
        raise ValueError('occ_targets_host: %d x %d labels do not fit 2^31' % (bs, voxel_num))
    rows = voxel_num // zdim
    where = None
    if row_table is not None:
        table = np.asarray(row_table).astype(np.int64)
        if table.shape != (rows, 3):
            raise ValueError('occ_targets_host: row_table must be [%d, 3], got %s' % (rows, table.shape))
        v = np.arange(voxel_num, dtype=np.int64)
        z, q = np.divmod(v, rows)
        where = ((bs * table[q, 0])[None, :] + np.arange(bs, dtype=np.int64)[:, None] * table[q, 1][None, :]
                 + table[q, 2][None, :]) * zdim + z[None, :]
        if bs and voxel_num and not np.array_equal(np.sort(where.reshape(-1)), np.arange(bs * voxel_num)):
            raise ValueError('occ_targets_host: row_table is no permutation of the label bytes')
    vol = np.full((bs, voxel_num), classes, dtype=np.uint8)
    count = np.zeros(bs + 1, dtype=np.int32)
    bad = np.zeros(2, dtype=np.int32)
    for b in range(bs):
        p = pairs[off[b]:off[b + 1]]
        ok = (p[:, 0] >= 0) & (p[:, 0] < voxel_num) & (p[:, 1] >= 0) & (p[:, 1] <= classes)
        bad[0] += int((~ok).sum())
        p = p[ok & (p[:, 1] < classes)]
        best = np.full(voxel_num, -1, dtype=np.int64)
        np.maximum.at(best, p[:, 0], p[:, 1])
        vol[b] = np.where(best >= 0, best, classes).astype(np.uint8)
        count[b] = int((best >= 0).sum())
        bad[1] += int((best[p[:, 0]] != p[:, 1]).sum())
    count[bs] = int(count[:bs].sum())
    if invalid is not None:
        inv = np.asarray(invalid).reshape(-1).astype(np.int64)
        ioff = _occ_offsets(invalid_offsets, inv.size, 'invalid_offsets')
        if ioff.size != bs + 1:
            raise ValueError('occ_targets_host: invalid_offsets must be [%d]' % (bs + 1))
        for b in range(bs):
            i = inv[ioff[b]:ioff[b + 1]]
            ok = (i >= 0) & (i < voxel_num)
            bad[0] += int((~ok).sum())
            vol[b, i[ok]] = 255
    if where is None:
        return vol.reshape(-1), count, bad
    labels = np.empty(bs * voxel_num, dtype=np.uint8)
    labels[where.reshape(-1)] = vol.reshape(-1)
    return labels, count, bad


class PackedOccGts:

    def __init__(self, buffer, bs, n_total, n_invalid, has_invalid, slot=None):
        self.buffer, self.bs, self.n_total, self.n_invalid, self.has_invalid = buffer, bs, n_total, n_invalid, has_invalid
        self._slot, self._generation = slot, (slot[2] if slot is not None else None)
        h = 2 * (bs + 1)
        self.offsets = buffer[:bs + 1]
        self.invalid_offsets = buffer[bs + 1:h] if has_invalid else None
        self.pairs = buffer[h:h + 2 * n_total].view(n_total, 2)
        self.invalid = buffer[h + 2 * n_total:h + 2 * n_total + n_invalid] if has_invalid else None

    def to(self, device):
        device = torch.device(device)
        if self._slot is not None and self._slot[2] != self._generation:
            raise RuntimeError('PackedOccGts.to: the staging buffer of this size class was packed again since -- one pack is '
                               'outstanding per size class: copy it (.to) before the next pack_occ_gts, or pack with pinned=False')
        if device.type != 'cuda':
            return PackedOccGts(self.buffer.clone(), self.bs, self.n_total, self.n_invalid, self.has_invalid)
        dev = self.buffer.to(device, non_blocking=True)
        if self._slot is not None:
            done = torch.cuda.Event()
            done.record()
            self._slot[1] = done
        return PackedOccGts(dev, self.bs, self.n_total, self.n_invalid, self.has_invalid)


_OCC_STAGING = {}


def pack_occ_gts(occ_gts, invalid=None, pinned=True):
    import numpy as np

    def arr(a, cols):
        if cols == 2 and isinstance(a, (list, tuple)):
            a = a[0]
        if a is None:
            return np.zeros((0, 2) if cols == 2 else (0,), dtype=np.int32)
        a = a.detach().cpu().numpy() if torch.is_tensor(a) else np.asarray(a)
        if a.size == 0:
            return np.zeros((0, 2) if cols == 2 else (0,), dtype=np.int32)
        if not np.issubdtype(a.dtype, np.integer):
            raise TypeError('pack_occ_gts: integer arrays expected, got %s' % a.dtype)
        if cols == 2 and (a.ndim != 2 or a.shape[1] != 2):
            raise ValueError('pack_occ_gts: a sample is [n, 2] (voxel index, class) pairs, got %s' % (a.shape,))
        return a if cols == 2 else a.reshape(-1)

    gts = [arr(a, 2) for a in occ_gts]
    bs = len(gts)
    has_invalid = invalid is not None
    inv = [arr(a, 1) for a in invalid] if has_invalid else []
    if has_invalid and len(inv) != bs:
        raise ValueError('pack_occ_gts: %d invalid lists for %d samples' % (len(inv), bs))
    n_total, n_invalid = sum(a.shape[0] for a in gts), sum(a.size for a in inv)
    used = 2 * (bs + 1) + 2 * n_total + n_invalid
    if max(n_total, n_invalid) >= 2 ** 31 - 1 or used >= 2 ** 31:
        raise ValueError('pack_occ_gts: %d pairs / %d invalid voxels exceed the int32 offsets' % (n_total, n_invalid))
    slot = None
    if pinned and torch.cuda.is_available():
        cap = 1024
        while cap < used:
            cap *= 2
        slot = _OCC_STAGING.get(cap)
        if slot is None:
            slot = _OCC_STAGING[cap] = [torch.empty(cap, dtype=torch.int32, pin_memory=True), None, 0]
        elif slot[1] is not None:
            slot[1].synchronize()
        slot[2] += 1
        host = slot[0][:used]
    else:
        host = torch.empty(used, dtype=torch.int32)
    hv = host.numpy()
    lim = np.iinfo(np.int32)

    def put(dst, a):
        if a.dtype.itemsize > 4 or a.dtype == np.uint32:
            np.clip(a, lim.min, lim.max, out=dst, casting='unsafe')
        else:
            dst[...] = a

    h = 2 * (bs + 1)
    hv[0] = 0
    hv[bs + 1] = 0
    if bs:
        hv[1:bs + 1] = np.cumsum([a.shape[0] for a in gts])
        hv[bs + 2:h] = np.cumsum([a.size for a in inv]) if has_invalid else 0
    pos = h
    for a in gts:
        put(hv[pos:pos + a.size].reshape(-1, 2), a)
        pos += a.size
    for a in inv:
        put(hv[pos:pos + a.size], a)
        pos += a.size
    return PackedOccGts(host, bs, n_total, n_invalid, has_invalid, slot)


def occ_targets(pairs, offsets, voxel_num, zdim, classes, row_table=None, invalid=None, invalid_offsets=None, out=None):
    what = 'occ_targets'
    pairs = _gpu(pairs, 'pairs')
    dev = pairs.device
    if pairs.dtype not in (torch.int32, torch.int64) or pairs.dim() != 2 or pairs.shape[1] != 2:
        raise TypeError('%s: pairs must be int32 or int64 [n_total, 2], got %s %s' % (what, pairs.dtype, tuple(pairs.shape)))

    def idx(t, name, shape):
        t = _gpu(t, name, torch.int32)
        if tuple(t.shape) != shape or t.device != dev:
            raise ValueError('%s: %s must be int32 %s on %s, got %s on %s' % (what, name, shape, dev, tuple(t.shape), t.device))
        return t

    if offsets.dim() != 1 or offsets.numel() < 1:
        raise ValueError('%s: offsets must be [bs + 1]' % what)
    bs = offsets.numel() - 1
    offsets = idx(offsets, 'offsets', (bs + 1,))
    voxel_num, zdim, classes = int(voxel_num), int(zdim), int(classes)
    if voxel_num < 0 or zdim < 1 or classes < 1:
        raise ValueError('%s: voxel_num=%d zdim=%d classes=%d' % (what, voxel_num, zdim, classes))
    if row_table is not None:
        row_table = idx(row_table, 'row_table', (voxel_num // zdim, 3))
    n_invalid = 0
    if (invalid is None) != (invalid_offsets is None):
        raise ValueError('%s: invalid and invalid_offsets come together' % what)
    if invalid is not None:
        invalid = _gpu(invalid, 'invalid')
        if invalid.dtype not in (torch.int32, torch.int64) or invalid.dim() != 1 or invalid.device != dev:
            raise TypeError('%s: invalid must be int32 or int64 [n_invalid] on %s' % (what, dev))
        invalid_offsets = idx(invalid_offsets, 'invalid_offsets', (bs + 1,))
        n_invalid = invalid.numel()
    total = bs * voxel_num
    padded = (total + 3) // 4 * 4
    if out is None:
        labels = torch.empty(padded, dtype=torch.uint8, device=dev)[:total]
        count = torch.empty(bs + 1, dtype=torch.int32, device=dev)
        bad = torch.empty(2, dtype=torch.int32, device=dev)
    else:
        labels, count, bad = out
        room = labels.untyped_storage().nbytes() - labels.storage_offset()
        if (labels.dtype != torch.uint8 or labels.numel() != total or not labels.is_contiguous() or labels.device != dev
                or room < padded):
            raise ValueError('%s: out labels must be %d contiguous uint8 on %s, allocated up to a multiple of 4 bytes' % (what, total, dev))
        labels = labels.view(-1)
        count, bad = idx(count, 'out count', (bs + 1,)), idx(bad, 'out bad', (2,))
    code = lambda t: 1 if t is not None and t.dtype == torch.int64 else 0
    _launch('ver_occ_targets', lambda: lib().ver_occ_targets(
        _p(pairs), code(pairs), _p(offsets), pairs.shape[0], _p(invalid), code(invalid), _p(invalid_offsets), n_invalid,
        _p(row_table), _p(labels), _p(count), _p(bad), voxel_num, zdim, classes, bs, _stream()))
    return labels, count, bad


def wgrad_tn_supported(a, g):
    return (a.is_cuda and g.is_cuda and a.dtype == torch.bfloat16 and g.dtype == torch.bfloat16 and a.dim() == 2
            and g.dim() == 2 and a.shape[0] == g.shape[0] and a.stride(1) == 1 and g.stride(1) == 1
            and a.stride(0) % 8 == 0 and g.stride(0) % 8 == 0 and a.data_ptr() % 16 == 0 and g.data_ptr() % 16 == 0
            and g.shape[1] % 4 == 0)


def wgrad_tn(a, g, out_dtype=None, splits=0, flags=0, out=None):
    if not wgrad_tn_supported(a, g):
        raise RuntimeError('wgrad_tn: unsupported operands %s %s / %s %s' % (tuple(a.shape), a.stride(), tuple(g.shape), g.stride()))
    m, ka = a.shape
    n = g.shape[1]
    out_dtype = out_dtype or a.dtype
    if out_dtype not in (torch.bfloat16, torch.float32):
        raise TypeError('wgrad_tn: out_dtype must be bf16 or fp32')
    L = lib()
    if splits <= 0:
        splits = L.ver_wgrad_tn_splits_ld(m, ka, n, max(a.stride(0), g.stride(0)))
    nbytes = L.ver_wgrad_tn_workspace(m, ka, n, splits)
    ws = torch.empty(nbytes // 4, dtype=torch.float32, device=a.device)
    if out is None:
        out = torch.empty(ka, n, dtype=out_dtype, device=a.device)
    elif not (out.is_cuda and out.shape == (ka, n) and out.dtype == out_dtype and out.stride(1) == 1):
        raise RuntimeError('wgrad_tn: out must be a [Ka, N] GPU matrix of out_dtype with unit column stride')
    _launch('ver_wgrad_tn', lambda: L.ver_wgrad_tn(
        _p(a), a.stride(0), _p(g), g.stride(0), m, ka, n, _p(out), out.stride(0), 1 if out_dtype == torch.bfloat16 else 0,
        splits, flags, _p(ws), nbytes, _stream()), meta=dict(flops=2.0 * m * ka * n))
    return out


def gemm_nn_supported(a, w):
    return (a.is_cuda and w.is_cuda and a.dtype == torch.bfloat16 and w.dtype == torch.bfloat16 and a.dim() == 2
            and w.dim() == 2 and a.shape[1] == w.shape[0] and a.stride(1) == 1 and w.stride(1) == 1
            and a.stride(0) % 8 == 0 and w.stride(0) % 8 == 0 and a.data_ptr() % 16 == 0 and w.data_ptr() % 16 == 0
            and a.shape[1] % 32 == 0 and a.shape[1] >= 64)


def gemm_nn_splits(m, k, n):
    return lib().ver_gemm_nn_splits(m, k, n)


def gemm_nn(a, w, bias=None, out=None, splits=None, timer_class='ver_gemm_nn'):
    if not gemm_nn_supported(a, w):
        raise RuntimeError('gemm_nn: unsupported operands %s %s / %s %s' % (tuple(a.shape), a.stride(), tuple(w.shape), w.stride()))
    m, k = a.shape
    n = w.shape[1]
    if out is None:
        out = torch.empty(m, n, dtype=torch.bfloat16, device=a.device)
    if out.shape != (m, n) or out.dtype != torch.bfloat16 or out.stride(1) != 1 or not out.is_cuda:
        raise RuntimeError('gemm_nn: out must be a bf16 [M, N] GPU matrix with unit column stride')
    if bias is not None:
        bias = _gpu(bias, 'bias').float().contiguous()
    if splits is None:
        splits = gemm_nn_splits(m, k, n)
    if splits > 1 and (n % 4 or out.stride(0) % 4 or out.data_ptr() % 8):
        splits = 1
    ws = torch.empty(splits * m * n, dtype=torch.float32, device=a.device) if splits > 1 else None
    _launch(timer_class, lambda: lib().ver_gemm_nn_splitk(
        _p(a), a.stride(0), _p(w), w.stride(0), _p(bias), _p(out), out.stride(0), m, k, n, splits, _p(ws),
        ws.numel() * 4 if ws is not None else 0, _stream()), meta=dict(flops=2.0 * m * k * n))
    return out


def gemm_nn_taps_supported(lattice, layout, w, c):
    return (lattice.is_cuda and lattice.dtype == torch.bfloat16 and lattice.is_contiguous() and layout in (PLAIN, ZSPLIT, PLANAR_ZSPLIT)
            and lattice.numel() * 2 < 2 ** 31 - 1 and c % 32 == 0 and c >= 64
            and (w is None or (w.is_cuda and w.dtype == torch.bfloat16 and w.dim() == 2 and w.stride(1) == 1 and w.stride(0) % 8 == 0
                               and w.data_ptr() % 16 == 0)))


def gemm_nn_taps(lattice, layout, combined_hw, taps, w, rowpos=None, bias=None, out=None, const_rows=None, planes=None,
                 timer_class='ver_gemm_nn'):
    lat, w = _gpu(lattice, 'lattice'), _gpu(w, 'w')
    plane_elems = nplanes = 0
    if planes is not None:
        nplanes, plane_elems = int(lat.shape[0]), int(lat[0].numel())
        if len(planes) != len(taps) or not lat.is_contiguous():
            raise ValueError('gemm_nn_taps: one source plane per tap, contiguous planes')
    lat_one = lat[0] if planes is not None else lat
    B, H, W, C, const_rows, ncst, cw, kdim, arr, ntaps = _segment_args(lat_one, layout, combined_hw, taps, const_rows, 'gemm_nn_taps')
    if not gemm_nn_taps_supported(lat_one, int(layout), w, C):
        raise RuntimeError('gemm_nn_taps: unsupported operands %s layout %d / %s %s' % (tuple(lat.shape), layout, tuple(w.shape), w.stride()))
    m, n = B * 2 * H * W, w.shape[1]
    if w.shape[0] != kdim:
        raise ValueError('gemm_nn_taps: w has %d rows, the segments span %d columns' % (w.shape[0], kdim))
    if out is None:
        out = torch.empty(m, n, dtype=torch.bfloat16, device=lat.device)
    if out.shape != (m, n) or out.dtype != torch.bfloat16 or out.stride(1) != 1 or not out.is_cuda:
        raise RuntimeError('gemm_nn_taps: out must be a bf16 [M, N] GPU matrix with unit column stride')
    if rowpos is not None:
        rowpos = _gpu(rowpos, 'rowpos').float().contiguous()
        if tuple(rowpos.shape) != (2 * H * W, n):
            raise ValueError('gemm_nn_taps: rowpos must be [2 H W, N]')
    if bias is not None:
        bias = _gpu(bias, 'bias').float().contiguous()
    parr = (ctypes.c_int * ntaps)(*[int(v) for v in planes]) if planes is not None else None
    _launch(timer_class, lambda: lib().ver_gemm_nn_planes(
        _p(lat), layout, B, H, W, C, plane_elems, nplanes, parr, arr, ntaps, _p(const_rows), ncst, cw, _p(w), w.stride(0),
        _p(rowpos), _p(bias), _p(out), out.stride(0), n, _stream()), meta=dict(flops=2.0 * m * w.shape[0] * n))
    return out


def _segment_args(lat, layout, combined_hw, taps, const_rows, name):
    H, W = combined_hw
    B, _, C = _lattice_dims(lat, int(layout))
    ncst = cw = 0
    if const_rows is not None:
        const_rows = _gpu(const_rows, 'const_rows')
        if not (const_rows.is_contiguous() and const_rows.dtype == torch.bfloat16 and const_rows.dim() == 3 and const_rows.shape[0] == 2 * H * W):
            raise ValueError('%s: const_rows must be a contiguous bf16 [2 H W, blocks, width] table' % name)
        ncst, cw = int(const_rows.shape[1]), int(const_rows.shape[2])
    taps = [((-1 - int(t[1]), 0, 0) if t[0] == 'c' else t) for t in taps]
    kdim = sum(cw if t[0] < 0 else C for t in taps)
    flat = [int(v) for t in taps for v in t]
    return B, H, W, C, const_rows, ncst, cw, kdim, (ctypes.c_int * len(flat))(*flat), len(taps)


WGRAD_SEGMENTS_ROWS = (16, 2048)


def wgrad_tn_segments_supported(lattice, layout, combined_hw, c, const_width, g):
    H, W = combined_hw
    return (WGRAD_SEGMENTS_ROWS[0] <= 2 * H * W <= WGRAD_SEGMENTS_ROWS[1]
            and lattice.is_cuda and lattice.dtype == torch.bfloat16 and lattice.is_contiguous() and layout in (PLAIN, ZSPLIT, PLANAR_ZSPLIT)
            and lattice.numel() * 2 < 2 ** 31 - 1 and c % 64 == 0 and const_width % 64 == 0
            and (g is None or (g.is_cuda and g.dtype == torch.bfloat16 and g.dim() == 2 and g.stride(1) == 1 and g.stride(0) % 8 == 0
                               and g.data_ptr() % 16 == 0 and g.shape[1] % 4 == 0)))


def wgrad_tn_segments(lattice, layout, combined_hw, taps, g, out_dtype=None, out=None, const_rows=None, splits=0):
    lat, g = _gpu(lattice, 'lattice'), _gpu(g, 'g')
    B, H, W, C, const_rows, ncst, cw, ka, arr, nseg = _segment_args(lat, layout, combined_hw, taps, const_rows, 'wgrad_tn_segments')
    if not wgrad_tn_segments_supported(lat, int(layout), (H, W), C, cw, g):
        raise RuntimeError('wgrad_tn_segments: unsupported operands %s layout %d / %s %s' % (tuple(lat.shape), layout, tuple(g.shape), g.stride()))
    if g.shape[0] != B * 2 * H * W:
        raise ValueError('wgrad_tn_segments: g has %d rows, %d cells' % (g.shape[0], B * 2 * H * W))
    n = g.shape[1]
    out_dtype = out_dtype or (out.dtype if out is not None else lat.dtype)
    if out is None:
        out = torch.empty(ka, n, dtype=out_dtype, device=lat.device)
    elif not (out.is_cuda and out.shape == (ka, n) and out.dtype == out_dtype and out.stride(1) == 1):
        raise RuntimeError('wgrad_tn_segments: out must be a [Ka, N] GPU matrix of out_dtype with unit column stride')
    L = lib()
    if splits <= 0:
        splits = L.ver_wgrad_tn_segments_splits(B, H, W, ka, n, g.stride(0))
    ws = torch.empty(splits * ka * n, dtype=torch.float32, device=lat.device)
    _launch('ver_wgrad_tn', lambda: L.ver_wgrad_tn_segments(
        _p(lat), layout, B, H, W, C, arr, nseg, _p(const_rows), ncst, cw, _p(g), g.stride(0), n, _p(out), out.stride(0),
        1 if out_dtype == torch.bfloat16 else 0, splits, _p(ws), ws.numel() * 4, _stream()), meta=dict(flops=2.0 * g.shape[0] * ka * n))
    return out
```

Measured before the change: 736.0.

## Batch four class wgrad GEMMs into one launch and fuse bias grad into wgrad

Adds a class-batched implicit wgrad kernel. It maps workgroups across the four upsample class products by tile range, so one launch with one split reduction replaces four separate launches. Separately, row_linear's backward now computes the bias gradient inside the wgrad GEMM: an extra MFMA against a ones vector on the first M-tile waves, with partial sums reduced in the same reduce kernel. This removes a separate g.sum pass over the gradient. The cost is more template variants, extra MFMAs and registers in the bias path, and a single split choice shared across classes.

```diff
diff --git a/include/ver_ops.h b/include/ver_ops.h
--- a/include/ver_ops.h
+++ b/include/ver_ops.h
@@ -205,6 +205,14 @@
                            int ncst, int cw, const void* g, long ldg, int N, void* out, long ldo, int out_dtype, int splits,
                            void* workspace, long workspace_bytes, void* stream);
 int  ver_wgrad_tn_segments_splits(int B, int H, int W, long Ka, int N, long ldg);
+int  ver_wgrad_tn_segments_classes(const void* lattice, int layout, int B, int H, int W, int C, const int* taps,
+                                   const int* class_nseg, const void* cst, int ncst, int cw, const void* g, long g_plane, long ldg,
+                                   int N, const int* class_row, void* out, long ldo, int out_dtype, int splits, void* workspace,
+                                   long workspace_bytes, void* stream);
+int  ver_wgrad_tn_segments_classes_splits(int B, int H, int W, const long* class_ka, int N, long ldg);
+long ver_wgrad_tn_bias_workspace(long M, int Ka, int N, int splits);
+int  ver_wgrad_tn_bias(const void* a, long lda, const void* g, long ldg, long M, int Ka, int N, void* out, long ldo, void* bias_out,
+                       int out_dtype, int splits, int flags, void* workspace, long workspace_bytes, void* stream);
 
 int  ver_gemm_nn(const void* a, long lda, const void* w, long ldw, const float* bias, void* c, long ldc, long M, int K,
                  int N, int flags, void* stream);
diff --git a/vln-ver_amd/csrc/ver_wgrad.hip b/vln-ver_amd/csrc/ver_wgrad.hip
--- a/vln-ver_amd/csrc/ver_wgrad.hip
+++ b/vln-ver_amd/csrc/ver_wgrad.hip
@@ -1,4 +1,6 @@
 #include "ver_gemm_tile.h"
+
+#include <type_traits>
 
 namespace {
 using namespace gemm_tile;
@@ -29,6 +31,23 @@
     signed char kind[64], dz[64], dy[64], dx[64];
 };
 
+struct WgradPlain {};
+struct WgradClasses {
+    long g_plane;
+    int tile_end[4];
+    int seg0[4], nseg[4];
+    int Ka[4], row[4];
+};
+struct WgradBias {
+    float* bias_out;
+    float* bias_ws;
+};
+template <typename Ext>
+struct WgradArgsExt {
+    WgradArgs p;
+    Ext e;
+};
+
 struct WTapLane {
     int taddr;
     int boff;
@@ -87,9 +106,10 @@
     int dmaoff;
 };
 
-template <int PS, int IMPL>
+template <int PS, int IMPL, bool BIAS>
 __device__ __forceinline__ void phase(char* lds, f32x4 (&acc)[8][4], const WgradLane& c, __amdgpu_buffer_rsrc_t ra,
-                                      __amdgpu_buffer_rsrc_t rg, unsigned& soA, unsigned& soG, const WgradArgs& t, WTapLane& tl) {
+                                      __amdgpu_buffer_rsrc_t rg, unsigned& soA, unsigned& soG, const WgradArgs& t, WTapLane& tl,
+                                      f32x4 (&bacc)[4], bool bias_on) {
     constexpr int SB = ((2 * PS) & 3) * kSlabBytes;
     constexpr int UP = 2 * PS >= 4 ? 65536 : 0;
     i32x2 al[8], ah[8], bl[4], bh[4];
@@ -138,6 +158,15 @@
 #pragma unroll
         for (int jt = 0; jt < 4; ++jt)
             acc[it][jt] = __builtin_amdgcn_mfma_f32_16x16x32_bf16(a[it], b[jt], acc[it][jt], 0, 0, 0);
+    if constexpr (BIAS) {
+        if (bias_on) {
+            bf16x8 ones;
+#pragma unroll
+            for (int i = 0; i < 8; ++i) ones[i] = (__bf16)1.0f;
+#pragma unroll
+            for (int jt = 0; jt < 4; ++jt) bacc[jt] = __builtin_amdgcn_mfma_f32_16x16x32_bf16(ones, b[jt], bacc[jt], 0, 0, 0);
+        }
+    }
     __builtin_amdgcn_s_setprio(0);
     __builtin_amdgcn_sched_barrier(0);
     if constexpr (IMPL >= 0) {
@@ -147,20 +176,22 @@
     __builtin_amdgcn_s_barrier();
 }
 
-template <int PS, int IMPL>
+template <int PS, int IMPL, bool BIAS>
 __device__ __forceinline__ void phases_from(int left, char* lds, f32x4 (&acc)[8][4], const WgradLane& c,
                                             __amdgpu_buffer_rsrc_t ra, __amdgpu_buffer_rsrc_t rg, unsigned& soA, unsigned& soG,
-                                            const WgradArgs& t, WTapLane& tl) {
+                                            const WgradArgs& t, WTapLane& tl, f32x4 (&bacc)[4], bool bias_on) {
     if constexpr (PS < kRing / kPhaseSlabs) {
         if (left > PS * kPhaseSlabs) {
-            phase<PS, IMPL>(lds, acc, c, ra, rg, soA, soG, t, tl);
-            phases_from<PS + 1, IMPL>(left, lds, acc, c, ra, rg, soA, soG, t, tl);
-        }
-    }
-}
-
-template <int IMPL>
-__device__ __forceinline__ void wgrad_body(const WgradArgs& p) {
+            phase<PS, IMPL, BIAS>(lds, acc, c, ra, rg, soA, soG, t, tl, bacc, bias_on);
+            phases_from<PS + 1, IMPL, BIAS>(left, lds, acc, c, ra, rg, soA, soG, t, tl, bacc, bias_on);
+        }
+    }
+}
+
+template <int IMPL, typename Ext>
+__device__ __forceinline__ void wgrad_body(const WgradArgs& p, const Ext& e) {
+    constexpr bool CLS = std::is_same<Ext, WgradClasses>::value, BIAS = std::is_same<Ext, WgradBias>::value;
+    static_assert(!CLS || IMPL >= 0, "classes: implicit A only");
     extern __shared__ __attribute__((aligned(1024))) char lds[];
     const int tid = threadIdx.x, lane = tid & 63;
     const int wave = __builtin_amdgcn_readfirstlane(tid >> 6);
@@ -177,14 +208,22 @@
             tile = b % p.T;
         }
     }
+    int Ka = p.Ka, seg_lo = 0, seg_hi = p.nseg, orow = 0;
+    const __bf16* G = p.G;
+    if constexpr (CLS) {
+        const int cls = (tile >= e.tile_end[0]) + (tile >= e.tile_end[1]) + (tile >= e.tile_end[2]);
+        if (cls) tile -= e.tile_end[cls - 1];
+        Ka = e.Ka[cls], seg_lo = e.seg0[cls], seg_hi = seg_lo + e.nseg[cls], orow = e.row[cls];
+        G += cls * e.g_plane;
+    }
     const int mt = tile / p.tiles_n, nt = tile - mt * p.tiles_n;
     const long row0 = (long)chunk * p.Mc;
     const long rows = max(0L, min(p.Mc, p.M - row0));
     const int nslab = (int)((rows + kSlabRows * kPhaseSlabs - 1) / (kSlabRows * kPhaseSlabs)) * kPhaseSlabs;
 
     const __bf16* ab = IMPL < 0 ? p.A + row0 * p.lda + (long)mt * kTile : nullptr;
-    const __bf16* gb = p.G + row0 * p.ldg + (long)nt * kTile;
-    const long abytes = ((p.M - row0 - 1) * p.lda + p.Ka - (long)mt * kTile) * 2;
+    const __bf16* gb = G + row0 * p.ldg + (long)nt * kTile;
+    const long abytes = ((p.M - row0 - 1) * p.lda + Ka - (long)mt * kTile) * 2;
     const long gbytes = ((p.M - row0 - 1) * p.ldg + p.N - (long)nt * kTile) * 2;
     const __amdgpu_buffer_rsrc_t rg = __builtin_amdgcn_make_buffer_rsrc((void*)gb, 0, (int)max(0L, min(gbytes, 0xFFFFFFFFL)), 0x00020000);
     WgradLane c;
@@ -195,8 +234,13 @@
         int* tables = reinterpret_cast<int*>(lds + kLdsBytes);
         auto seg_of = [&](int col0) {
             int seg = -1;
-            for (int i = 0; i < p.nseg; ++i)
-                if (col0 >= p.seg_start[i] && col0 < p.seg_start[i + 1]) seg = i;
+            if constexpr (CLS) {
+                for (int i = seg_lo; i < seg_hi; ++i)
+                    if (col0 >= p.seg_start[i] && col0 < Ka) seg = i;
+            } else {
+                for (int i = 0; i < p.nseg; ++i)
+                    if (col0 >= p.seg_start[i] && col0 < p.seg_start[i + 1]) seg = i;
+            }
             return seg;
         };
         for (int q = 0; q < 4; ++q) {
@@ -251,6 +295,13 @@
 #pragma unroll
             for (int r = 0; r < Shape::NR; ++r) acc[it][jt][r] = 0.0f;
 
+    f32x4 bacc[4];
+    const bool bias_on = BIAS && mt == 0 && wr == 0;
+#pragma unroll
+    for (int jt = 0; jt < 4; ++jt)
+#pragma unroll
+        for (int r = 0; r < 4; ++r) bacc[jt][r] = 0.0f;
+
 #pragma unroll
     for (int s = 0; s < kAhead; ++s) {
         if constexpr (IMPL < 0) {
@@ -281,12 +332,20 @@
     if (wr == 1) __builtin_amdgcn_s_barrier();
 
     int s = 0;
-    for (; s + kRing <= nslab; s += kRing) phases_from<0, IMPL>(kRing, lds, acc, c, ra, rg, soA, soG, p, tl);
-    phases_from<0, IMPL>(nslab - s, lds, acc, c, ra, rg, soA, soG, p, tl);
+    for (; s + kRing <= nslab; s += kRing) phases_from<0, IMPL, BIAS>(kRing, lds, acc, c, ra, rg, soA, soG, p, tl, bacc, bias_on);
+    phases_from<0, IMPL, BIAS>(nslab - s, lds, acc, c, ra, rg, soA, soG, p, tl, bacc, bias_on);
     if (wr == 0) __builtin_amdgcn_s_barrier();
     asm volatile("s_waitcnt vmcnt(0)" ::: "memory");
 
     const int i0 = mt * kTile + 128 * wr + Shape::lane_row(lane), j0 = nt * kTile + 64 * wc + (lane & (Shape::TW - 1));
+    if constexpr (BIAS) {
+        if (bias_on && lane < Shape::TW) {
+            float* dst = p.S == 1 && p.out ? e.bias_out : e.bias_ws + (long)chunk * p.N;
+#pragma unroll
+            for (int jt = 0; jt < 4; ++jt)
+                if (j0 + Shape::TW * jt < p.N) dst[j0 + Shape::TW * jt] = bacc[jt][0];
+        }
+    }
     if (p.S == 1 && p.out) {
 #pragma unroll
         for (int it = 0; it < Shape::NI; ++it)
@@ -296,17 +355,17 @@
 #pragma unroll
                 for (int r = 0; r < Shape::NR; ++r) {
                     const int i = i0 + Shape::TW * it + Shape::reg_row(r);
-                    if (i < p.Ka && j < p.N) {
+                    if (i < Ka && j < p.N) {
                         if (p.out_bf16)
-                            reinterpret_cast<__bf16*>(p.out)[(long)i * p.ldo + j] = (__bf16)acc[it][jt][r];
+                            reinterpret_cast<__bf16*>(p.out)[(long)(orow + i) * p.ldo + j] = (__bf16)acc[it][jt][r];
                         else
-                            reinterpret_cast<float*>(p.out)[(long)i * p.ldo + j] = acc[it][jt][r];
+                            reinterpret_cast<float*>(p.out)[(long)(orow + i) * p.ldo + j] = acc[it][jt][r];
                     }
                 }
             }
         return;
     }
-    float* out = p.ws + (long)chunk * p.Ka * p.N;
+    float* out = p.ws + ((long)chunk * p.Ka + orow) * p.N;
 #pragma unroll
     for (int it = 0; it < Shape::NI; ++it)
 #pragma unroll
@@ -315,26 +374,35 @@
 #pragma unroll
             for (int r = 0; r < Shape::NR; ++r) {
                 const int i = i0 + Shape::TW * it + Shape::reg_row(r);
-                if (i < p.Ka && j < p.N) out[(long)i * p.N + j] = acc[it][jt][r];
+                if (i < Ka && j < p.N) out[(long)i * p.N + j] = acc[it][jt][r];
             }
         }
 }
 
 __global__ __launch_bounds__(512) void k_wgrad_tn(WgradArgs p) {
-    wgrad_body<-1>(p);
+    wgrad_body<-1>(p, WgradPlain{});
+}
+
+__global__ __launch_bounds__(512) void k_wgrad_tn_bias(WgradArgsExt<WgradBias> a) {
+    wgrad_body<-1>(a.p, a.e);
 }
 
 template <int L>
 __global__ __launch_bounds__(512) void k_wgrad_tn_seg(WgradArgs p) {
-    wgrad_body<L>(p);
+    wgrad_body<L>(p, WgradPlain{});
+}
+
+template <int L>
+__global__ __launch_bounds__(512) void k_wgrad_tn_seg_classes(WgradArgsExt<WgradClasses> a) {
+    wgrad_body<L>(a.p, a.e);
 }
 
 template <typename OT>
-__global__ __launch_bounds__(256) void k_wgrad_reduce(const float* __restrict__ ws, OT* __restrict__ out, long ldo, int S,
-                                                      int Ka, int N) {
+__device__ __forceinline__ void wgrad_reduce_body(const float* __restrict__ ws, OT* __restrict__ out, long ldo, int S, int Ka, int N,
+                                                  unsigned nblocks) {
     const long n4 = (long)Ka * N / 4;
     const long stride = (long)Ka * N;
-    for (long e = blockIdx.x * 256L + threadIdx.x; e < n4; e += (long)gridDim.x * 256) {
+    for (long e = blockIdx.x * 256L + threadIdx.x; e < n4; e += (long)nblocks * 256) {
         float4 acc = *reinterpret_cast<const float4*>(ws + 4 * e);
         for (int s = 1; s < S; ++s) {
             const float4 v = *reinterpret_cast<const float4*>(ws + s * stride + 4 * e);
@@ -359,15 +427,35 @@
     }
 }
 
+template <typename OT>
+__global__ __launch_bounds__(256) void k_wgrad_reduce(const float* __restrict__ ws, OT* __restrict__ out, long ldo, int S,
+                                                      int Ka, int N) {
+    wgrad_reduce_body(ws, out, ldo, S, Ka, N, gridDim.x);
+}
+
+template <typename OT>
+__global__ __launch_bounds__(256) void k_wgrad_reduce_bias(const float* __restrict__ ws, OT* __restrict__ out, long ldo, int S,
+                                                           int Ka, int N, int nblocks, const float* __restrict__ wsb,
+                                                           float* __restrict__ bias) {
+    if ((int)blockIdx.x < nblocks) {
+        wgrad_reduce_body(ws, out, ldo, S, Ka, N, (unsigned)nblocks);
+        return;
+    }
+    const int j = ((int)blockIdx.x - nblocks) * 256 + threadIdx.x;
+    if (j >= N) return;
+    float acc = wsb[j];
+    for (int s = 1; s < S; ++s) acc += wsb[(long)s * N + j];
+    bias[j] = acc;
+}
+
 long max_chunk_rows(long ld) {
     if (ld <= 0) return 45000;
     const long rows = (0xFFFFFFFFL / (ld * 2)) - 16 * kRing - 2 * kSlabRows - 1;
     return rows < 45000 ? (rows > 2 * kSlabRows ? rows : 2 * kSlabRows) : 45000;
 }
 
-int pick_splits(long M, int Ka, int N, long ld = 0) {
+int pick_splits_tiles(long M, long tiles, long Ka, int N, long ld) {
     const long cap = max_chunk_rows(ld);
-    const long tiles = (long)((Ka + kTile - 1) / kTile) * ((N + kTile - 1) / kTile);
     static const int cand[] = {1, 2, 3, 4, 6, 8, 12, 16, 24, 32, 48, 64};
     int best = 0;
     double best_us = 0.0;
@@ -391,16 +479,22 @@
     return best;
 }
 
+int pick_splits(long M, int Ka, int N, long ld = 0) {
+    return pick_splits_tiles(M, (long)((Ka + kTile - 1) / kTile) * ((N + kTile - 1) / kTile), Ka, N, ld);
+}
+
 int launch_wgrad(const char* who, WgradArgs& p, int layout, long M, long Ka, int N, void* out, long ldo, int out_dtype, int splits,
-                 void* workspace, long workspace_bytes, hipStream_t st) {
+                 void* workspace, long workspace_bytes, hipStream_t st, const WgradClasses* cls = nullptr, long tiles = 0,
+                 float* bias_out = nullptr) {
     const long ld = p.lda > p.ldg ? p.lda : p.ldg;
-    const int S = splits > 0 ? splits : pick_splits(M, (int)Ka, N, ld);
+    const int S = splits > 0 ? splits : cls ? pick_splits_tiles(M, tiles, Ka, N, ld) : pick_splits(M, (int)Ka, N, ld);
     VER_REQUIRE(S <= 65536, VER_EINVAL, "%s: %d row chunks", who, S);
     const long Mc = ((M + S - 1) / S + 2 * kSlabRows - 1) / (2 * kSlabRows) * (2 * kSlabRows);
     VER_REQUIRE((Mc + 16 * kRing) * ld * 2 < 0xFFFFFFFFL, VER_EUNSUPPORTED,
                 "%s: a row chunk exceeds the 4-GiB range of a buffer offset (more splits)", who);
-    VER_REQUIRE(workspace_bytes >= (long)S * Ka * N * (long)sizeof(float), VER_EINVAL, "%s: workspace of %ld bytes, %ld needed", who,
-                workspace_bytes, (long)S * Ka * N * (long)sizeof(float));
+    const long ws_rows = bias_out ? Ka + 1 : Ka;
+    VER_REQUIRE(workspace_bytes >= (long)S * ws_rows * N * (long)sizeof(float), VER_EINVAL, "%s: workspace of %ld bytes, %ld needed", who,
+                workspace_bytes, (long)S * ws_rows * N * (long)sizeof(float));
     p.ws = (float*)workspace;
     p.M = M;
     p.Mc = Mc;
@@ -408,23 +502,39 @@
     p.Ka = (int)Ka;
     p.N = N;
     p.tiles_n = (N + kTile - 1) / kTile;
-    p.T = (int)((Ka + kTile - 1) / kTile) * p.tiles_n;
+    p.T = cls ? (int)tiles : (int)((Ka + kTile - 1) / kTile) * p.tiles_n;
+    VER_REQUIRE((long)p.T * S < 0x7FFFFFFFL, VER_EUNSUPPORTED, "%s: %ld workgroups", who, (long)p.T * S);
+    float* bias_ws = (float*)workspace + (long)S * Ka * N;
     const bool direct = S == 1 && M > 0;
     p.out = direct ? out : nullptr;
     p.ldo = ldo;
     p.out_bf16 = out_dtype == VER_BF16;
     if (M > 0) {
-        const auto kern = layout < 0 ? k_wgrad_tn : layout == 0 ? k_wgrad_tn_seg<0> : layout == 2 ? k_wgrad_tn_seg<2> : k_wgrad_tn_seg<3>;
         const int ldsb = layout < 0 ? kLdsBytes : kLdsBytes + 4 * p.P * 4;
-        if (int rc = launch_tile_kernel(who, kern, p, p.T * S, ldsb, st)) return rc;
-    } else if (int zrc = ver_zero_async(workspace, (size_t)S * Ka * N * sizeof(float), st)) {
+        if (cls) {
+            const auto kern = layout == 0 ? k_wgrad_tn_seg_classes<0> : layout == 2 ? k_wgrad_tn_seg_classes<2> : k_wgrad_tn_seg_classes<3>;
+            if (int rc = launch_tile_kernel(who, kern, WgradArgsExt<WgradClasses>{p, *cls}, p.T * S, ldsb, st)) return rc;
+        } else if (bias_out) {
+            if (int rc = launch_tile_kernel(who, k_wgrad_tn_bias, WgradArgsExt<WgradBias>{p, {bias_out, bias_ws}}, p.T * S, ldsb, st)) return rc;
+        } else {
+            const auto kern = layout < 0 ? k_wgrad_tn : layout == 0 ? k_wgrad_tn_seg<0> : layout == 2 ? k_wgrad_tn_seg<2> : k_wgrad_tn_seg<3>;
+            if (int rc = launch_tile_kernel(who, kern, p, p.T * S, ldsb, st)) return rc;
+        }
+    } else if (int zrc = ver_zero_async(workspace, (size_t)S * ws_rows * N * sizeof(float), st)) {
         return zrc;
     }
     if (direct) return ver_check_launch(who);
     const long n4 = Ka * N / 4;
     long grid = (n4 + 255) / 256;
     if (grid > 8192) grid = 8192;
-    if (out_dtype == VER_F32)
+    const unsigned gridb = (unsigned)(grid + (N + 255) / 256);
+    if (bias_out && out_dtype == VER_F32)
+        hipLaunchKernelGGL(k_wgrad_reduce_bias<float>, dim3(gridb), dim3(256), 0, st, (const float*)workspace, (float*)out, ldo, S, (int)Ka, N,
+                           (int)grid, (const float*)bias_ws, bias_out);
+    else if (bias_out)
+        hipLaunchKernelGGL(k_wgrad_reduce_bias<__bf16>, dim3(gridb), dim3(256), 0, st, (const float*)workspace, (__bf16*)out, ldo, S, (int)Ka, N,
+                           (int)grid, (const float*)bias_ws, bias_out);
+    else if (out_dtype == VER_F32)
         hipLaunchKernelGGL(k_wgrad_reduce<float>, dim3((unsigned)grid), dim3(256), 0, st, (const float*)workspace, (float*)out, ldo, S, (int)Ka, N);
     else
         hipLaunchKernelGGL(k_wgrad_reduce<__bf16>, dim3((unsigned)grid), dim3(256), 0, st, (const float*)workspace, (__bf16*)out, ldo, S, (int)Ka, N);
@@ -448,23 +558,46 @@
     return (long)splits * Ka * N * (long)sizeof(float);
 }
 
-extern "C" int ver_wgrad_tn(const void* a, long lda, const void* g, long ldg, long M, int Ka, int N, void* out, long ldo,
-                            int out_dtype, int splits, int flags, void* workspace, long workspace_bytes, void* stream) {
-    VER_REQUIRE(M >= 0 && Ka > 0 && N > 0, VER_EINVAL, "ver_wgrad_tn: bad sizes M=%ld Ka=%d N=%d", M, Ka, N);
-    VER_REQUIRE(out && workspace && ((a && g) || M == 0), VER_EINVAL, "ver_wgrad_tn: null pointer argument");
-    VER_REQUIRE(out_dtype == VER_F32 || out_dtype == VER_BF16, VER_EINVAL, "ver_wgrad_tn: out_dtype %d", out_dtype);
-    VER_REQUIRE(flags == 0, VER_EINVAL, "ver_wgrad_tn: unknown flags 0x%x", flags);
-    VER_REQUIRE(lda >= Ka && ldg >= N && ldo >= N, VER_EINVAL, "ver_wgrad_tn: row pitch smaller than the row");
+namespace {
+int wgrad_tn_entry(const char* who, const void* a, long lda, const void* g, long ldg, long M, int Ka, int N, void* out, long ldo,
+                   float* bias_out, int out_dtype, int splits, int flags, void* workspace, long workspace_bytes, void* stream) {
+    VER_REQUIRE(M >= 0 && Ka > 0 && N > 0, VER_EINVAL, "%s: bad sizes M=%ld Ka=%d N=%d", who, M, Ka, N);
+    VER_REQUIRE(out && workspace && ((a && g) || M == 0), VER_EINVAL, "%s: null pointer argument", who);
+    VER_REQUIRE(out_dtype == VER_F32 || out_dtype == VER_BF16, VER_EINVAL, "%s: out_dtype %d", who, out_dtype);
+    VER_REQUIRE(flags == 0, VER_EINVAL, "%s: unknown flags 0x%x", who, flags);
+    VER_REQUIRE(lda >= Ka && ldg >= N && ldo >= N, VER_EINVAL, "%s: row pitch smaller than the row", who);
     VER_REQUIRE(lda % 8 == 0 && ldg % 8 == 0 && ((uintptr_t)a & 15) == 0 && ((uintptr_t)g & 15) == 0, VER_EUNSUPPORTED,
-                "ver_wgrad_tn: operands must be 16-byte aligned with row pitches that are multiples of 8 elements");
+                "%s: operands must be 16-byte aligned with row pitches that are multiples of 8 elements", who);
     VER_REQUIRE(N % 4 == 0 && ldo % 4 == 0 && ((uintptr_t)out & 15) == 0, VER_EUNSUPPORTED,
-                "ver_wgrad_tn: N and the output pitch must be multiples of 4");
+                "%s: N and the output pitch must be multiples of 4", who);
     WgradArgs p = {};
     p.A = (const __bf16*)a;
     p.G = (const __bf16*)g;
     p.lda = lda;
     p.ldg = ldg;
-    return launch_wgrad("ver_wgrad_tn", p, -1, M, Ka, N, out, ldo, out_dtype, splits, workspace, workspace_bytes, (hipStream_t)stream);
+    return launch_wgrad(who, p, -1, M, Ka, N, out, ldo, out_dtype, splits, workspace, workspace_bytes, (hipStream_t)stream, nullptr, 0,
+                        bias_out);
+}
+}
+
+extern "C" int ver_wgrad_tn(const void* a, long lda, const void* g, long ldg, long M, int Ka, int N, void* out, long ldo,
+                            int out_dtype, int splits, int flags, void* workspace, long workspace_bytes, void* stream) {
+    return wgrad_tn_entry("ver_wgrad_tn", a, lda, g, ldg, M, Ka, N, out, ldo, nullptr, out_dtype, splits, flags, workspace,
+                          workspace_bytes, stream);
+}
+
+extern "C" long ver_wgrad_tn_bias_workspace(long M, int Ka, int N, int splits) {
+    if (Ka <= 0 || N <= 0) return 0;
+    if (splits <= 0) splits = ver_wgrad_tn_splits(M, Ka, N);
+    return (long)splits * (Ka + 1L) * N * (long)sizeof(float);
+}
+
+extern "C" int ver_wgrad_tn_bias(const void* a, long lda, const void* g, long ldg, long M, int Ka, int N, void* out, long ldo,
+                                 void* bias_out, int out_dtype, int splits, int flags, void* workspace, long workspace_bytes,
+                                 void* stream) {
+    VER_REQUIRE(bias_out, VER_EINVAL, "ver_wgrad_tn_bias: null pointer argument");
+    return wgrad_tn_entry("ver_wgrad_tn_bias", a, lda, g, ldg, M, Ka, N, out, ldo, (float*)bias_out, out_dtype, splits, flags, workspace,
+                          workspace_bytes, stream);
 }
 
 extern "C" int ver_wgrad_tn_segments(const void* lattice, int layout, int B, int H, int W, int C, const int* taps, int nseg,
@@ -514,3 +647,90 @@
     if (M <= 0 || Ka <= 0 || N <= 0) return 1;
     return pick_splits(M, (int)Ka, N, ldg);
 }
+
+namespace {
+bool class_tiles(const long* ka, int N, long* tiles, long* ka_sum) {
+    *tiles = *ka_sum = 0;
+    for (int c = 0; c < 4; ++c) {
+        if (ka[c] <= 0) return false;
+        *tiles += (ka[c] + kTile - 1) / kTile * ((N + kTile - 1) / kTile);
+        *ka_sum += ka[c];
+    }
+    return true;
+}
+}
+
+extern "C" int ver_wgrad_tn_segments_classes_splits(int B, int H, int W, const long* class_ka, int N, long ldg) {
+    const long M = (long)B * 2 * H * W;
+    long tiles, ka_sum;
+    if (M <= 0 || N <= 0 || !class_ka || !class_tiles(class_ka, N, &tiles, &ka_sum)) return 1;
+    return pick_splits_tiles(M, tiles, ka_sum, N, ldg);
+}
+
+extern "C" int ver_wgrad_tn_segments_classes(const void* lattice, int layout, int B, int H, int W, int C, const int* taps,
+                                             const int* class_nseg, const void* cst, int ncst, int cw, const void* g, long g_plane,
+                                             long ldg, int N, const int* class_row, void* out, long ldo, int out_dtype, int splits,
+                                             void* workspace, long workspace_bytes, void* stream) {
+    const char* who = "ver_wgrad_tn_segments_classes";
+    VER_REQUIRE(class_nseg && class_row, VER_EINVAL, "%s: null pointer argument", who);
+    long nseg = 0;
+    for (int c = 0; c < 4; ++c) {
+        VER_REQUIRE(class_nseg[c] > 0, VER_EINVAL, "%s: class %d has no segment", who, c);
+        nseg += class_nseg[c];
+    }
+    VER_REQUIRE(nseg <= 64, VER_EUNSUPPORTED, "%s: %ld segments in the four classes (at most 64)", who, nseg);
+    if (int rc = check_lattice_args(who, layout, B, H, W, C, N, (int)nseg)) return rc;
+    VER_REQUIRE(out && workspace && ((lattice && g && taps) || B == 0), VER_EINVAL, "%s: null pointer argument", who);
+    VER_REQUIRE(out_dtype == VER_F32 || out_dtype == VER_BF16, VER_EINVAL, "%s: out_dtype %d", who, out_dtype);
+    VER_REQUIRE(C % 64 == 0 && (cst == nullptr || (ncst > 0 && ncst <= 64 && cw > 0 && cw % 64 == 0 && ((uintptr_t)cst & 15) == 0)),
+                VER_EUNSUPPORTED, "%s: segment widths (C = %d, pattern blocks of %d) must be multiples of 64", who, C, cw);
+    const long M = (long)B * 2 * H * W, lbytes = (long)B * 4 * H * W * C * 2;
+    const int P = 2 * H * W;
+    VER_REQUIRE(P >= kSlabRows && P <= 2048 && lbytes < 0x7FFFFFFFL, VER_EUNSUPPORTED,
+                "%s: %d rows per viewpoint / a source lattice of %ld bytes (16 <= rows <= 2048, below 2 GiB)", who, P, lbytes);
+    VER_REQUIRE(ldg >= N && ldo >= N && ldg % 8 == 0 && g_plane % 8 == 0 && g_plane >= 0 && ((uintptr_t)g & 15) == 0 &&
+                    ((uintptr_t)lattice & 15) == 0,
+                VER_EUNSUPPORTED, "%s: g must be 16-byte aligned with a row pitch and a plane stride that are multiples of 8 elements", who);
+    VER_REQUIRE(N % 4 == 0 && ldo % 4 == 0 && ((uintptr_t)out & 15) == 0, VER_EUNSUPPORTED,
+                "%s: N and the output pitch must be multiples of 4", who);
+    WgradArgs p = {};
+    WgradClasses e = {};
+    long ka[4], tiles, ka_sum;
+    for (int c = 0, s0 = 0; c < 4; s0 += class_nseg[c], ++c) {
+        if (int rc = check_segments(who, who, taps + 3 * s0, class_nseg[c], C, cst, ncst, cw, &ka[c])) return rc;
+        VER_REQUIRE(ka[c] < 0x7FFFFFFFL, VER_EUNSUPPORTED, "%s: %ld columns", who, ka[c]);
+        for (int i = s0, col = 0; i < s0 + class_nseg[c]; ++i) {
+            const int dz = taps[3 * i];
+            p.seg_start[i] = col;
+            p.kind[i] = dz < 0;
+            p.dz[i] = (signed char)(dz < 0 ? -1 - dz : dz);
+            if (dz >= 0) p.dy[i] = (signed char)taps[3 * i + 1], p.dx[i] = (signed char)taps[3 * i + 2];
+            col += dz < 0 ? cw : C;
+        }
+        e.seg0[c] = s0, e.nseg[c] = class_nseg[c], e.Ka[c] = (int)ka[c], e.row[c] = class_row[c];
+    }
+    class_tiles(ka, N, &tiles, &ka_sum);
+    VER_REQUIRE(ka_sum < 0x7FFFFFFFL && tiles < 0x7FFFFFFFL, VER_EUNSUPPORTED, "%s: %ld columns", who, ka_sum);
+    for (int c = 0; c < 4; ++c) {
+        VER_REQUIRE(class_row[c] >= 0 && class_row[c] + ka[c] <= ka_sum, VER_EINVAL, "%s: class %d: rows %d .. outside the %ld stacked rows",
+                    who, c, class_row[c], ka_sum);
+        for (int d = 0; d < c; ++d)
+            VER_REQUIRE(class_row[c] >= class_row[d] + ka[d] || class_row[d] >= class_row[c] + ka[c], VER_EINVAL,
+                        "%s: the rows of classes %d and %d overlap", who, d, c);
+    }
+    for (int c = 0, t = 0; c < 4; ++c) {
+        t += (int)((ka[c] + kTile - 1) / kTile) * ((N + kTile - 1) / kTile);
+        e.tile_end[c] = t;
+    }
+    e.g_plane = g_plane;
+    p.nseg = (int)nseg;
+    p.G = (const __bf16*)g;
+    p.ldg = ldg;
+    p.lattice = (const __bf16*)lattice;
+    p.lattice_bytes = lbytes;
+    p.cst = (const __bf16*)cst;
+    p.cst_bytes = cst ? (long)P * ncst * cw * 2 : 0;
+    p.B = B, p.H = H, p.W = W, p.C = C, p.P = P, p.CW = cw, p.ncst = ncst;
+    return launch_wgrad(who, p, layout, M, ka_sum, N, out, ldo, out_dtype, splits, workspace, workspace_bytes, (hipStream_t)stream, &e,
+                        tiles);
+}
diff --git a/vln-ver_amd/dense_heads/row_linear.py b/vln-ver_amd/dense_heads/row_linear.py
--- a/vln-ver_amd/dense_heads/row_linear.py
+++ b/vln-ver_amd/dense_heads/row_linear.py
@@ -2,6 +2,7 @@
 import torch.nn.functional as F
 
 _CHUNK = 8000
+_BIAS_IN_WGRAD = True
 
 
 class _RowLinear(torch.autograd.Function):
@@ -23,9 +24,16 @@
         n, o = g.shape
         gx = g @ w if ctx.needs_input_grad[0] else None
         gb = None
+        own = g.dtype == torch.bfloat16 and x.dtype == torch.bfloat16 and n >= 4096 and min(o, x.shape[1]) >= 192
+        if own and ctx.has_bias and _BIAS_IN_WGRAD:
+            from ..hipops import wgrad_tn, wgrad_tn_supported
+            if wgrad_tn_supported(x, g):
+                wide = torch.float32 if ctx.weight_dtype == torch.float32 else torch.bfloat16
+                gwt, gb = wgrad_tn(x, g, out_dtype=wide, bias=True)
+                return gx, gwt.t(), gb.to(torch.bfloat16) if wide == torch.bfloat16 else gb
         if ctx.has_bias:
             gb = g.sum(0, dtype=torch.float32)
-        if g.dtype == torch.bfloat16 and x.dtype == torch.bfloat16 and n >= 4096 and min(o, x.shape[1]) >= 192:
+        if own:
             from ..hipops import wgrad_tn, wgrad_tn_supported
             if wgrad_tn_supported(g, x):
                 wide = torch.float32 if ctx.weight_dtype == torch.float32 else torch.bfloat16
diff --git a/vln-ver_amd/dense_heads/upsample.py b/vln-ver_amd/dense_heads/upsample.py
--- a/vln-ver_amd/dense_heads/upsample.py
+++ b/vln-ver_amd/dense_heads/upsample.py
@@ -411,11 +411,14 @@
             d_a = operand.new_empty(m, kt)
             d_a[:, kt - _PW2:] = 0
         d_stack = operand.new_empty(n_rows, 2 * co)
+        if ctx.implicit:
+            from ..hipops import WgradClassBatch
+            batch = WgradClassBatch(g, d_stack)
         for p, (cls, (c0, c1, r0, r1)) in enumerate(zip(_CLASSES, ranges)):
             if ctx.implicit:
                 from ..hipops import wgrad_tn_segments
                 wgrad_tn_segments(operand, layout, (hc, wc), _class_segments_z4(cls, ci), g[p], out=d_stack[r0:r1],
-                                  const_rows=_const_rows_z4(ci, hc, wc, operand.device, dt)[0])
+                                  const_rows=_const_rows_z4(ci, hc, wc, operand.device, dt)[0], batch=batch)
             else:
                 _dgrad_class(d_a, p, g[p], stack[r0:r1], c0, c1)
                 rows_tn(operand[:, c0:c1], g[p], out=d_stack[r0:r1])
diff --git a/vln-ver_amd/hipops.py b/vln-ver_amd/hipops.py
--- a/vln-ver_amd/hipops.py
+++ b/vln-ver_amd/hipops.py
@@ -1841,7 +1841,7 @@
             and g.shape[1] % 4 == 0)
 
 
-def wgrad_tn(a, g, out_dtype=None, splits=0, flags=0, out=None):
+def wgrad_tn(a, g, out_dtype=None, splits=0, flags=0, out=None, bias=False):
     if not wgrad_tn_supported(a, g):
         raise RuntimeError('wgrad_tn: unsupported operands %s %s / %s %s' % (tuple(a.shape), a.stride(), tuple(g.shape), g.stride()))
     m, ka = a.shape
@@ -1852,12 +1852,18 @@
     L = lib()
     if splits <= 0:
         splits = L.ver_wgrad_tn_splits_ld(m, ka, n, max(a.stride(0), g.stride(0)))
-    nbytes = L.ver_wgrad_tn_workspace(m, ka, n, splits)
+    nbytes = (L.ver_wgrad_tn_bias_workspace if bias else L.ver_wgrad_tn_workspace)(m, ka, n, splits)
     ws = torch.empty(nbytes // 4, dtype=torch.float32, device=a.device)
     if out is None:
         out = torch.empty(ka, n, dtype=out_dtype, device=a.device)
     elif not (out.is_cuda and out.shape == (ka, n) and out.dtype == out_dtype and out.stride(1) == 1):
         raise RuntimeError('wgrad_tn: out must be a [Ka, N] GPU matrix of out_dtype with unit column stride')
+    if bias:
+        db = torch.empty(n, dtype=torch.float32, device=a.device)
+        _launch('ver_wgrad_tn', lambda: L.ver_wgrad_tn_bias(
+            _p(a), a.stride(0), _p(g), g.stride(0), m, ka, n, _p(out), out.stride(0), _p(db), 1 if out_dtype == torch.bfloat16 else 0,
+            splits, flags, _p(ws), nbytes, _stream()), meta=dict(flops=2.0 * m * ka * n))
+        return out, db
     _launch('ver_wgrad_tn', lambda: L.ver_wgrad_tn(
         _p(a), a.stride(0), _p(g), g.stride(0), m, ka, n, _p(out), out.stride(0), 1 if out_dtype == torch.bfloat16 else 0,
         splits, flags, _p(ws), nbytes, _stream()), meta=dict(flops=2.0 * m * ka * n))
@@ -1963,7 +1969,23 @@
                                and g.data_ptr() % 16 == 0 and g.shape[1] % 4 == 0)))
 
 
-def wgrad_tn_segments(lattice, layout, combined_hw, taps, g, out_dtype=None, out=None, const_rows=None, splits=0):
+class WgradClassBatch:
+
+    def __init__(self, g, out):
+        self.g, self.out, self.taps, self.rows = g, out, [], []
+
+
+def wgrad_tn_segments(lattice, layout, combined_hw, taps, g, out_dtype=None, out=None, const_rows=None, splits=0, batch=None):
+    if batch is not None:
+        c, pitch = len(batch.taps), batch.out.stride(0) * batch.out.element_size()
+        off = out.data_ptr() - batch.out.data_ptr()
+        if c >= 4 or g.data_ptr() != batch.g[c].data_ptr() or g.shape != batch.g[c].shape or off % pitch or out.stride() != batch.out.stride():
+            raise ValueError('wgrad_tn_segments: product %d is not plane %d of the batch\'s g / a row range of its result' % (c, c))
+        batch.taps.append(taps)
+        batch.rows.append(off // pitch)
+        if c == 3:
+            wgrad_tn_segments_classes(lattice, layout, combined_hw, batch.taps, batch.g, batch.out, batch.rows, const_rows=const_rows, splits=splits)
+        return out
     lat, g = _gpu(lattice, 'lattice'), _gpu(g, 'g')
     B, H, W, C, const_rows, ncst, cw, ka, arr, nseg = _segment_args(lat, layout, combined_hw, taps, const_rows, 'wgrad_tn_segments')
     if not wgrad_tn_segments_supported(lat, int(layout), (H, W), C, cw, g):
@@ -1984,3 +2006,31 @@
         _p(lat), layout, B, H, W, C, arr, nseg, _p(const_rows), ncst, cw, _p(g), g.stride(0), n, _p(out), out.stride(0),
         1 if out_dtype == torch.bfloat16 else 0, splits, _p(ws), ws.numel() * 4, _stream()), meta=dict(flops=2.0 * g.shape[0] * ka * n))
     return out
+
+
+def wgrad_tn_segments_classes(lattice, layout, combined_hw, class_taps, g, out, class_rows, const_rows=None, splits=0):
+    lat, g = _gpu(lattice, 'lattice'), _gpu(g, 'g')
+    if len(class_taps) != 4 or len(class_rows) != 4:
+        raise ValueError('wgrad_tn_segments_classes: four segment lists and four first rows')
+    parts = [_segment_args(lat, layout, combined_hw, taps, const_rows, 'wgrad_tn_segments_classes') for taps in class_taps]
+    B, H, W, C, const_rows, ncst, cw = parts[0][:7]
+    kas = [p[7] for p in parts]
+    flat = [v for p in parts for v in p[8]]
+    if g.dim() != 3 or g.shape[0] != 4 or not g.is_contiguous() or \
+            not wgrad_tn_segments_supported(lat, int(layout), (H, W), C, cw, g[0]):
+        raise RuntimeError('wgrad_tn_segments_classes: unsupported operands %s layout %d / %s %s' % (tuple(lat.shape), layout, tuple(g.shape), g.stride()))
+    if g.shape[1] != B * 2 * H * W:
+        raise ValueError('wgrad_tn_segments_classes: g has %d rows per class, %d cells' % (g.shape[1], B * 2 * H * W))
+    n = g.shape[2]
+    if not (out.is_cuda and out.shape == (sum(kas), n) and out.dtype in (torch.bfloat16, torch.float32) and out.stride(1) == 1):
+        raise RuntimeError('wgrad_tn_segments_classes: out must be a [sum Ka, N] bf16 / fp32 GPU matrix with unit column stride')
+    L = lib()
+    if splits <= 0:
+        splits = L.ver_wgrad_tn_segments_classes_splits(B, H, W, (ctypes.c_long * 4)(*kas), n, g.stride(1))
+    ws = torch.empty(splits * sum(kas) * n, dtype=torch.float32, device=lat.device)
+    _launch('ver_wgrad_tn', lambda: L.ver_wgrad_tn_segments_classes(
+        _p(lat), layout, B, H, W, C, (ctypes.c_int * len(flat))(*flat), (ctypes.c_int * 4)(*[p[9] for p in parts]), _p(const_rows),
+        ncst, cw, _p(g), g.stride(0), g.stride(1), n, (ctypes.c_int * 4)(*[int(r) for r in class_rows]), _p(out), out.stride(0),
+        1 if out.dtype == torch.bfloat16 else 0, splits, _p(ws), ws.numel() * 4, _stream()),
+        meta=dict(flops=2.0 * g.shape[1] * sum(kas) * n))
+    return out
```

Result: no change. 738.4 (median of 6 runs) (+0.3%).
